# xguo7/SND-VAE

Measured on AMD Instinct MI355X. Metric: training graphs/sec + ELBO-step ms, N=4096 d=64, at 1/2/4/8 MI355X, higher is better.
Workload: dtype bf16; 1 GPU; C2: node-latent SND-VAE train step, N=4096, d=64, 8 graphs/GPU, HIP-graph replay; n_nodes=4096, latent=64, graphs_per_gpu=8, global_batch=8, parallelism=dp1, hip_graph=True

## Files before the change

snd_vae_amd/csrc/snd_fast.hip:

```cpp
#include "snd_fast.hpp"
#include "snd_gather.hpp"
#include "snd_pack.hpp"

#include <algorithm>

namespace snd {

namespace {

constexpr int NT = 256;

typedef short v4s __attribute__((ext_vector_type(4)));
typedef short v8s __attribute__((ext_vector_type(8)));
typedef __attribute__((address_space(3))) v4s lds_v4s;

__device__ __forceinline__ int swz(int row, int kp) {
  return kp >= 128 ? (row & 15) : (kp == 64 ? ((row >> 1) & 7) : 0);
}

__device__ __forceinline__ uint4 pack8(float4 lo, float4 hi) {
  bf16x8 v;
  v[0] = (__bf16)lo.x; v[1] = (__bf16)lo.y; v[2] = (__bf16)lo.z; v[3] = (__bf16)lo.w;
  v[4] = (__bf16)hi.x; v[5] = (__bf16)hi.y; v[6] = (__bf16)hi.z; v[7] = (__bf16)hi.w;
  return __builtin_bit_cast(uint4, v);
}

struct PackPack { PackDesc d[kMaxPack]; };

__global__ void __launch_bounds__(NT) pack_kernel(PackPack pk) {
  const PackDesc& d = pk.d[blockIdx.y];
  const int nch = pack_chunks(d);
  for (int i = blockIdx.x * NT + threadIdx.x; i < nch; i += gridDim.x * NT) pack_chunk(d, i);
}

typedef __attribute__((address_space(1))) const void* gptr_t;
typedef __attribute__((address_space(3))) void* lptr_t;

__device__ __forceinline__ void glds16(const void* g, void* lds_base) {
  __builtin_amdgcn_global_load_lds((gptr_t)g, (lptr_t)lds_base, 16, 0, 0);
}

__device__ __forceinline__ void glds16_async(const void* g, void* lds_base) {
  const unsigned dst = __builtin_amdgcn_readfirstlane((unsigned)(uintptr_t)(lptr_t)lds_base);
  unsigned keep;
  asm volatile("s_mov_b32 %0, m0\n\ts_mov_b32 m0, %2\n\ts_nop 0\n\t"
               "global_load_lds_dwordx4 %1, off\n\ts_mov_b32 m0, %0"
               : "=&s"(keep) : "v"(g), "s"(dst) : "memory");
}

__device__ __forceinline__ int rc_xchunks(int T, int lkc) {
  return (((kRcRows + T - 1) << lkc) + 63) & ~63;
}

constexpr int RCT = 1024;

template <int EPI> struct RcNcp { static constexpr int v = 0; };
template <> struct RcNcp<RC_LIN> { static constexpr int v = 1; };
template <> struct RcNcp<RC_DECBWD> { static constexpr int v = 3; };
template <> struct RcNcp<RC_ENC1> { static constexpr int v = 4; };
template <> struct RcNcp<RC_ENC0> { static constexpr int v = 2; };

template <int EPI, int NBH>
__global__ void __launch_bounds__(RCT) rowconv_kernel(RcArgs a) {
  extern __shared__ __attribute__((aligned(16))) __bf16 lds[];
  __shared__ __attribute__((aligned(16))) float cps[8][RcNcp<EPI>::v > 0 ? RcNcp<EPI>::v : 1][128];
  __shared__ float colp[8][128];
  constexpr int NCP = RcNcp<EPI>::v;
  const int T = a.T, H = (T - 1) >> 1, kp = a.kp, np = a.np;
  const int lkc = kp == 256 ? 5 : (kp == 128 ? 4 : (kp == 64 ? 3 : 2));
  const int XR = kRcRows + T - 1;
  const int xch = rc_xchunks(T, lkc);
  __bf16* xs = lds;
  __bf16* ws = lds + (xch << 3);
  const int tid = threadIdx.x, lane = tid & 63, w = tid >> 6;
  const int li = lane & 15, lg = lane >> 4;
  const int rb = w & 7, nb0 = NBH * (w >> 3);
  int tb = blockIdx.x;
  if (EPI == RC_ENC0 && a.g_rowptr && a.npg % kRcRows == 0 && (a.R / a.npg) % 8 == 0) {
    const int tpg = a.npg / kRcRows, x = tb & 7, sq = tb >> 3, g8 = sq / tpg;
    tb = (x + 8 * g8) * tpg + (sq - g8 * tpg);
  }
  const int r0 = tb * kRcRows;
  const int rend = min(r0 + kRcRows, a.R);
  const int nbase = blockIdx.y * a.npb;
  const int nloc = min(a.npb, np - nbase);
  const int nbc = nloc >> 4;
  const bool use_cp = NCP > 0 && a.colpart != nullptr && !(kdbg(a.dbg) & 64);

  if (!(kdbg(a.dbg) & 1)) {
    const int segc = (nloc * kp) >> 9, npc = T * segc;
    const char* g = reinterpret_cast<const char*>(a.wpk) + lane * 16;
    for (int j = w; j < npc; j += RCT / 64) {
      const int t = j / segc, jj = j - t * segc;
      glds16(g + ((long long)(t * np + nbase) * kp * 2) + (jj << 10), reinterpret_cast<char*>(ws) + (j << 10));
    }
  }
  if (tid < nloc) {
    const int nl = tid, n = nbase + tid;
    const bool cv = n < a.N && a.cols.valid(n) && !(kdbg(a.dbg) & 16);
    const bool pa = n < a.cols.a;
    const int ia = pa ? n : a.cols.logical(n), ib = n - a.cols.offb;
    auto par = [&](const float* A, const float* Bv) {
      return !cv || !A ? 0.f : (pa || !Bv ? A[ia] : Bv[ib]);
    };
    colp[0][nl] = par(a.bias, a.bias_b);
    colp[1][nl] = par(a.gamma, a.gamma_b) * kBnC;
    colp[2][nl] = par(a.beta, a.beta_b);
    if constexpr (EPI == RC_ENC1) {
      colp[3][nl] = (cv && n < a.h) ? a.g2[n] * kBnC : 0.f;
      colp[4][nl] = (cv && n < a.h) ? a.b2[n] : 0.f;
    }
    if constexpr (EPI == RC_ENC0) {
#pragma unroll
      for (int k = 0; k < 4; ++k) colp[3 + k][nl] = (cv && k < a.f) ? a.w0[k * a.N + n] : 0.f;
    }
    if constexpr (EPI == RC_LIN || EPI == RC_FWD) {
#pragma unroll
      for (int k = 0; k < 4; ++k) colp[3 + k][nl] = (cv && k < a.ktail) ? a.wtail[k * a.ldwt + n] : 0.f;
    }
  }

  unsigned cvm[NBH];
#pragma unroll
  for (int i = 0; i < NBH; ++i) {
    cvm[i] = 0u;
#pragma unroll
    for (int e = 0; e < 4; ++e) {
      const int n = nbase + 16 * (nb0 + i) + 4 * lg + e;
      if (nb0 + i < nbc && n < a.N && a.cols.valid(n)) cvm[i] |= 1u << e;
    }
  }
  const int wsw = swz(li, kp);

  int s0 = r0;
  bool first = true;
  while (s0 < rend) {
    int glo, ghi, s1;
    if (T == 1) {
      glo = r0; ghi = rend; s1 = rend;
    } else {
      const int gs = (s0 / a.npg) * a.npg;
      glo = gs; ghi = min(a.R, gs + a.npg); s1 = min(rend, ghi);
    }
    if (!first) __syncthreads();
    bool gathered = false;
    if constexpr (EPI == RC_ENC0 && NBH <= 2) {
      if (a.g_rowptr) {
        gathered = true;
        const int rs = tid >> 3, sub = tid & 7;
        const int gr = r0 + rs;
        float acc8[8] = {0.f, 0.f, 0.f, 0.f, 0.f, 0.f, 0.f, 0.f};
        if (gr < rend) {
          const __amdgpu_buffer_rsrc_t rsx = rows_rsrc(a.x, (long long)a.R * a.ldx * 2);
          gather_rows16<1>(a.g_colidx, a.g_rowptr[gr], a.g_rowptr[gr + 1], rsx, 2u * a.ldx, sub,
                           [&](int, const u32x4 (&v)[1], bool) { acc8v(acc8, v[0]); });
        }
        const uint4 o = to_bf16x8(acc8);
        *reinterpret_cast<uint4*>(xs + rs * kp + ((sub ^ swz(rs, kp)) << 3)) = o;
        if (gr < rend && 8 * sub < a.K)
          *reinterpret_cast<uint4*>(reinterpret_cast<__bf16*>(a.gout) + (long long)gr * a.ldgo + 8 * sub) = o;
      }
    }
    if (!gathered && !(kdbg(a.dbg) & 2)) {
      const int kc = 1 << lkc;
      for (int j = w; j < (xch >> 6); j += RCT / 64) {
        const int q = (j << 6) + lane;
        const int row = q >> lkc, pc = q & (kc - 1);
        const int c = pc ^ swz(row, kp);
        const int gr = r0 - H + row;
        const bool v = row < XR && gr >= glo && gr < ghi && 8 * c < a.K;
        const void* g = v ? (const void*)(reinterpret_cast<const __bf16*>(a.x) + (long long)gr * a.ldx + 8 * c)
                          : (const void*)a.zero;
        glds16(g, reinterpret_cast<char*>(xs) + (j << 10));
      }
    }
    const int r = r0 + 16 * rb + li;
    const bool rv = r >= s0 && r < s1;
    f32x4 ypf[NBH];
#pragma unroll
    for (int i = 0; i < NBH; ++i) ypf[i] = f32x4{0.f, 0.f, 0.f, 0.f};
    if constexpr (EPI == RC_DECBWD || EPI == RC_ENC1) {
      if (rv && !(kdbg(a.dbg) & 32)) {
#pragma unroll
        for (int i = 0; i < NBH; ++i) {
          const int n0 = nbase + 16 * (nb0 + i) + 4 * lg;
          if constexpr (EPI == RC_DECBWD) {
            const float* yp = a.y + (long long)r * a.ldy + n0;
            if (cvm[i] == 15u) ypf[i] = *reinterpret_cast<const f32x4*>(yp);
            else
#pragma unroll
              for (int e = 0; e < 4; ++e) if (cvm[i] >> e & 1u) ypf[i][e] = yp[e];
          } else {
            if (NBH <= 3 && cvm[i] == 15u && n0 + 3 < a.h && (a.ldp & 3) == 0 &&
                (reinterpret_cast<uintptr_t>(a.p) & 15) == 0) {
              ypf[i] = *reinterpret_cast<const f32x4*>(a.p + (long long)r * a.ldp + n0);
            } else {
#pragma unroll
              for (int e = 0; e < 4; ++e) {
                const int n = n0 + e;
                if (cvm[i] >> e & 1u)
                  ypf[i][e] = n < a.h ? a.p[(long long)r * a.ldp + n] : a.xf[(long long)r * a.ldxf + (n - a.h)];
              }
            }
          }
        }
      }
    }
    float ax[4] = {0.f, 0.f, 0.f, 0.f};
    if constexpr (EPI == RC_ENC0) {
      if (rv)
#pragma unroll
        for (int k = 0; k < 4; ++k) if (k < a.f) ax[k] = a.p[(long long)r * a.ldp + k];
    }
    if constexpr (EPI == RC_LIN || EPI == RC_FWD) {
      if (rv && a.ktail > 0) {
        const __bf16* xt = reinterpret_cast<const __bf16*>(a.x) + (long long)r * a.ldx + a.K;
#pragma unroll
        for (int k = 0; k < 4; ++k) if (k < a.ktail) ax[k] = (float)xt[k];
      }
    }
    __builtin_amdgcn_s_waitcnt(0x0F70);
    __syncthreads();

    f32x4 acc[NBH];
#pragma unroll
    for (int i = 0; i < NBH; ++i) acc[i] = f32x4{0.f, 0.f, 0.f, 0.f};
    const int kcs = (kdbg(a.dbg) & 4) ? 0 : kp >> 5;
    for (int t = 0; t < T; ++t) {
      const int xrow = 16 * rb + li + t;
      const __bf16* xrp = xs + xrow * kp;
      const int xsw = swz(xrow, kp);
      const __bf16* wrp = ws + (t * nloc + li) * kp;
      for (int ks = 0; ks < kcs; ++ks) {
        const int ch = 4 * ks + lg;
        const bf16x8 bx = *reinterpret_cast<const bf16x8*>(xrp + ((ch ^ xsw) << 3));
#pragma unroll
        for (int i = 0; i < NBH; ++i) {
          if (nb0 + i < nbc) {
            const bf16x8 aw = *reinterpret_cast<const bf16x8*>(
                wrp + 16 * (nb0 + i) * kp + ((ch ^ wsw) << 3));
            acc[i] = __builtin_amdgcn_mfma_f32_16x16x32_bf16(aw, bx, acc[i], 0, 0, 0);
          }
        }
      }
    }

#pragma unroll
    for (int i = 0; i < NBH; ++i) {
      const int nb = nb0 + i;
      if (nb >= nbc || (kdbg(a.dbg) & 128)) continue;
      const int nl0 = 16 * nb + 4 * lg, n0 = nbase + nl0;
      const unsigned cm = rv ? cvm[i] : 0u;
      float o[4], qs[NCP > 0 ? NCP : 1][4];
#pragma unroll
      for (int q = 0; q < (NCP > 0 ? NCP : 1); ++q)
#pragma unroll
        for (int e = 0; e < 4; ++e) qs[q][e] = 0.f;
      const float4 bia = *reinterpret_cast<const float4*>(&colp[0][nl0]);
      const float4 gam = *reinterpret_cast<const float4*>(&colp[1][nl0]);
      const float4 bet = *reinterpret_cast<const float4*>(&colp[2][nl0]);
      const float bi[4] = {bia.x, bia.y, bia.z, bia.w};
      if constexpr (EPI == RC_LIN || EPI == RC_FWD) {
        if (a.ktail > 0)
#pragma unroll
          for (int e = 0; e < 4; ++e)
#pragma unroll
            for (int k = 0; k < 4; ++k) acc[i][e] += ax[k] * colp[3 + k][nl0 + e];
      }
      const float ga[4] = {gam.x, gam.y, gam.z, gam.w};
      const float be[4] = {bet.x, bet.y, bet.z, bet.w};
      unsigned sm = cm;
      if constexpr (EPI == RC_LIN) {
#pragma unroll
        for (int e = 0; e < 4; ++e) { o[e] = acc[i][e] + bi[e]; qs[0][e] = (cm >> e & 1u) ? o[e] : 0.f; }
      } else if constexpr (EPI == RC_FWD) {
        float yv[4];
#pragma unroll
        for (int e = 0; e < 4; ++e) { yv[e] = acc[i][e] + bi[e]; o[e] = lrelu(yv[e] * ga[e] + be[e]); }
        float* yp = a.y + (long long)r * a.ldy + n0;
        if (kdbg(a.dbg) & 8) {
        } else if (cm == 15u) *reinterpret_cast<float4*>(yp) = make_float4(yv[0], yv[1], yv[2], yv[3]);
        else
#pragma unroll
          for (int e = 0; e < 4; ++e) if (cm >> e & 1u) yp[e] = yv[e];
      } else if constexpr (EPI == RC_DECBWD) {
#pragma unroll
        for (int e = 0; e < 4; ++e) {
          const float yv = ypf[i][e];
          const float dt = (cm >> e & 1u) ? acc[i][e] * lrelu_grad(yv * ga[e] + be[e]) : 0.f;
          o[e] = dt * ga[e];
          qs[0][e] = dt * yv;
          qs[1][e] = dt;
          qs[2][e] = o[e];
        }
      } else if constexpr (EPI == RC_ENC1) {
#pragma unroll
        for (int e = 0; e < 4; ++e) {
          const int n = n0 + e, nl = nl0 + e;
          const bool ok = cm >> e & 1u;
          const float dg = ok ? acc[i][e] : 0.f;
          const bool bpart = n < a.h;
          const float pv = ypf[i][e];
          const float a1 = lrelu(pv);
          const float x2 = bpart ? a1 * colp[3][nl] + colp[4][nl] : pv;
          qs[0][e] = dg * x2;
          qs[1][e] = dg;
          const float dh2 = dg * ga[e];
          o[e] = 0.f;
          qs[2][e] = 0.f;
          qs[3][e] = 0.f;
          if (bpart) {
            qs[2][e] = dh2 * a1;
            qs[3][e] = dh2;
            o[e] = dh2 * colp[3][nl] * lrelu_grad(pv);
          } else {
            sm &= ~(1u << e);
          }
        }
      } else {
#pragma unroll
        for (int e = 0; e < 4; ++e) {
          float pv = 0.f;
#pragma unroll
          for (int k = 0; k < 4; ++k) pv += ax[k] * colp[3 + k][nl0 + e];
          const float db = (cm >> e & 1u) ? acc[i][e] : 0.f;
          qs[0][e] = db * lrelu(pv);
          qs[1][e] = db;
          o[e] = db * ga[e] * lrelu_grad(pv);
        }
      }
      if (kdbg(a.dbg) & 8) sm = 0u;
      if (a.out_bf16) {
        __bf16* op = reinterpret_cast<__bf16*>(a.out) + (long long)r * a.ldo + n0;
        if (sm == 15u) {
          bf16x4 v4;
#pragma unroll
          for (int e = 0; e < 4; ++e) v4[e] = (__bf16)o[e];
          *reinterpret_cast<bf16x4*>(op) = v4;
        } else {
#pragma unroll
          for (int e = 0; e < 4; ++e) if (sm >> e & 1u) op[e] = (__bf16)o[e];
        }
      } else {
        float* op = reinterpret_cast<float*>(a.out) + (long long)r * a.ldo + n0;
        if (sm == 15u) *reinterpret_cast<float4*>(op) = make_float4(o[0], o[1], o[2], o[3]);
        else
#pragma unroll
          for (int e = 0; e < 4; ++e) if (sm >> e & 1u) op[e] = o[e];
      }
      if constexpr (NCP > 0) {
        if (use_cp) {
#pragma unroll
          for (int q = 0; q < NCP; ++q) {
            float v[4];
#pragma unroll
            for (int e = 0; e < 4; ++e) v[e] = row16_sum(qs[q][e]);
            if (li == 0) {
              float4* cp = reinterpret_cast<float4*>(&cps[rb][q][nl0]);
              if (first) *cp = make_float4(v[0], v[1], v[2], v[3]);
              else { float4 o4 = *cp; o4.x += v[0]; o4.y += v[1]; o4.z += v[2]; o4.w += v[3]; *cp = o4; }
            }
          }
        }
      }
    }
    s0 = s1;
    first = false;
  }
  if constexpr (NCP > 0) {
    if (use_cp) {
      __syncthreads();
      for (int i = tid; i < NCP * nloc; i += RCT) {
        const int q = i / nloc, nl = i - q * nloc, n = nbase + nl;
        if (n >= a.N) continue;
        float t = 0.f;
#pragma unroll
        for (int b = 0; b < 8; ++b) t += cps[b][q][nl];
        a.colpart[((long long)tb * NCP + q) * a.N + n] = t;
      }
    }
  }
}

__device__ __forceinline__ bf16x8 tr_pair(const __bf16* p0, const __bf16* p1) {
  const v4s lo = __builtin_amdgcn_ds_read_tr16_b64_v4i16((lds_v4s*)(p0));
  const v4s hi = __builtin_amdgcn_ds_read_tr16_b64_v4i16((lds_v4s*)(p1));
  const v8s c = __builtin_shufflevector(lo, hi, 0, 1, 2, 3, 4, 5, 6, 7);
  return __builtin_bit_cast(bf16x8, c);
}

__device__ __forceinline__ int trsw(int row, int kp) {
  return kp == 128 ? (((row & 3) << 1) | (row & 8))
                   : (kp == 64 ? ((row & 2) | ((row & 8) >> 1)) : (((row >> 3) & 1) << 1));
}
__device__ __forceinline__ int log2kc(int kp) { return kp == 128 ? 4 : (kp == 64 ? 3 : 2); }

__device__ __forceinline__ void stage_tr_image(const __bf16* src, int ld, int K, int base, int nrows,
                                               int vlo, int vhi, int kp, __bf16* dst,
                                               const void* zero) {
  const int lane = threadIdx.x & 63, w = threadIdx.x >> 6;
  const int lk = log2kc(kp), kc = 1 << lk;
  const int npc = ((nrows << lk) + 63) >> 6;
  for (int j = w; j < npc; j += 4) {
    const int q = (j << 6) + lane;
    const int row = q >> lk, pc = q & (kc - 1);
    const int c = pc ^ trsw(row, kp);
    const int gr = base + row;
    const bool v = row < nrows && gr >= vlo && gr < vhi && 8 * c < K;
    const void* g = v ? (const void*)(src + (long long)gr * ld + 8 * c) : zero;
    glds16(g, reinterpret_cast<char*>(dst) + (j << 10));
  }
}

__device__ __forceinline__ int tr_off(int row, int col, int kp) {
  const int c = col >> 3;
  return row * kp + (((c ^ trsw(row, kp)) << 3) | (col & 4));
}

constexpr int WGT = 1024;

__device__ __forceinline__ int cdiv_d(int a, int b) { return (a + b - 1) / b; }

struct WgUnit { int sub, s0, s1, glo, ghi; };

__device__ __forceinline__ WgUnit wg_unit(const WgArgs& a, int sub, int s0, int c1) {
  const int send = min(c1, sub + kRcRows);
  WgUnit u;
  u.sub = sub; u.s0 = s0;
  if (a.T == 1) { u.glo = sub; u.ghi = send; u.s1 = send; }
  else {
    const int gs = (s0 / a.npg) * a.npg;
    u.glo = gs; u.ghi = min(a.R, gs + a.npg); u.s1 = min(send, u.ghi);
  }
  return u;
}

constexpr int kWgStampWords = 12;
__device__ __forceinline__ void wg_stamp(unsigned* ts, int i, bool on) {
  if (on && threadIdx.x == 0 && i < kWgStampWords) ts[i] = (unsigned)__builtin_amdgcn_s_memrealtime();
}

template <int NBO, int NPW = 1>
__device__ __forceinline__ void wgrad_body(const WgArgs& a, const int bx, const int by, __bf16* lds,
                                           unsigned* tsp = nullptr) {
  const bool stamp = tsp != nullptr;
  const int T = a.T, H = (T - 1) >> 1;
  const int XR = kRcRows + T - 1;
  const int kpx = a.K <= 32 ? 32 : (a.K <= 64 ? 64 : 128);
  const int kpy = a.N <= 32 ? 32 : (a.N <= 64 ? 64 : 128);
  const int xch = ((XR << log2kc(kpx)) + 63) & ~63;
  const int bufe = (xch << 3) + kRcRows * kpy;
  const int tid = threadIdx.x, lane = tid & 63, w = __builtin_amdgcn_readfirstlane(tid >> 6);
  const int li = lane & 15, lg = lane >> 4, tq = li >> 2, tp = li & 3;
  const __bf16* xg = reinterpret_cast<const __bf16*>(a.x);
  const __bf16* dg = reinterpret_cast<const __bf16*>(a.dy);
  const int c0 = bx * a.rows_per_wg, c1 = min(a.R, c0 + a.rows_per_wg);
  auto stage = [&](const WgUnit& u, int b) __attribute__((always_inline)) {
    if (kdbg(a.dbg) & 2) return;
    __bf16* xs = lds + b * bufe;
    __bf16* ds = xs + (xch << 3);
    const int lkx = log2kc(kpx), lky = log2kc(kpy);
    const int npx = xch >> 6, npy = (kRcRows << lky) >> 6;
    for (int j = w; j < npx + npy; j += WGT / 64) {
      const bool isx = j < npx;
      const int jj = isx ? j : j - npx;
      const int lk = isx ? lkx : lky, kp = isx ? kpx : kpy;
      const int q = (jj << 6) + lane;
      const int row = q >> lk, pc = q & ((1 << lk) - 1);
      const int c = pc ^ trsw(row, kp);
      const void* g = a.zero;
      if (isx) {
        const int gr = u.sub - H + row;
        if (row < XR && gr >= u.glo && gr < u.ghi && 8 * c < a.K) g = xg + (long long)gr * a.ldx + 8 * c;
      } else {
        const int gr = u.sub + row;
        if (gr >= u.s0 && gr < u.s1 && 8 * c < a.N) g = dg + (long long)gr * a.lddy + 8 * c;
      }
      glds16_async(g, reinterpret_cast<char*>(isx ? xs : ds) + (jj << 10));
    }
  };

  const WgUnit u0 = wg_unit(a, c0, c0, c1);
  if (c0 < c1) stage(u0, 0);
  const int cbn = (a.K + 15) >> 4;
  const int P = T * cbn;
  bool pvs[NPW];
  int ts[NPW], cbs[NPW];
#pragma unroll
  for (int i = 0; i < NPW; ++i) {
    const int wl = w + 16 * i, p = by * a.pairs_per_wg + wl;
    pvs[i] = wl < a.pairs_per_wg && p < P;
    ts[i] = pvs[i] ? p / cbn : 0;
    cbs[i] = pvs[i] ? p - ts[i] * cbn : 0;
  }
  const bool pv = pvs[0];

  f32x4 acc[NPW][NBO];
#pragma unroll
  for (int i = 0; i < NPW; ++i)
#pragma unroll
    for (int j = 0; j < NBO; ++j) acc[i][j] = f32x4{0.f, 0.f, 0.f, 0.f};

  const int rk0 = 8 * lg + tq;
  int xoff[NPW], xoff2[NPW];
#pragma unroll
  for (int i = 0; i < NPW; ++i) {
    xoff[i] = tr_off(rk0 + ts[i], 16 * cbs[i] + 4 * tp, kpx);
    xoff2[i] = tr_off(rk0 + ts[i] + 4, 16 * cbs[i] + 4 * tp, kpx);
  }
  if (kdbg(a.dbg) & 32) return;
  const int doff = rk0 * kpy;
  const int swd = trsw(rk0, kpy), tpl = (4 * tp) & 4, tph = tp >> 1;
  wg_stamp(tsp, 2, stamp);
  if (c0 < c1) {
    WgUnit u = u0;
    for (int k = 0;; ++k) {
      __builtin_amdgcn_s_waitcnt(0x0F70);
      __syncthreads();
      wg_stamp(tsp, 3 + k, stamp && k < 6);
      int nsub = u.sub, ns0 = u.s1;
      if (ns0 >= min(c1, u.sub + kRcRows)) { nsub = u.sub + kRcRows; ns0 = nsub; }
      const bool more = nsub < c1;
      WgUnit un{};
      if (more) { un = wg_unit(a, nsub, ns0, c1); stage(un, (k + 1) & 1); }
      const __bf16* xs = lds + (k & 1) * bufe;
      const __bf16* ds = xs + (xch << 3);
      if (!(kdbg(a.dbg) & 4) && pv) {
#pragma unroll
        for (int ks = 0; ks < kRcRows / 32; ++ks) {
          const __bf16* xb = xs + 32 * ks * kpx;
          const __bf16* db = ds + doff + 32 * ks * kpy;
          bf16x8 bxv[NPW];
#pragma unroll
          for (int i = 0; i < NPW; ++i) bxv[i] = tr_pair(xb + xoff[i], xb + xoff2[i]);
#pragma unroll
          for (int ob = 0; ob < NBO; ++ob) {
            const int dob = (((2 * ob + tph) ^ swd) << 3) | tpl;
            const bf16x8 af = tr_pair(db + dob, db + dob + 4 * kpy);
#pragma unroll
            for (int i = 0; i < NPW; ++i)
              if (i == 0 || pvs[i]) acc[i][ob] = __builtin_amdgcn_mfma_f32_16x16x32_bf16(af, bxv[i], acc[i][ob], 0, 0, 0);
          }
        }
      }
      if (!more) break;
      u = un;
    }
  }
  if (kdbg(a.dbg) & 8) return;
  const int sK = a.sK, sn4 = a.sn4;
#pragma unroll
  for (int i = 0; i < NPW; ++i) {
    const int k = 16 * cbs[i] + li;
    if (!pvs[i] || k >= a.K) continue;
    float* row = a.slab + (long long)bx * T * sK * sn4 + ((long long)ts[i] * sK + a.wk0 + k) * sn4 + a.wn0;
#pragma unroll
    for (int ob = 0; ob < NBO; ++ob) {
      const int n0 = 16 * ob + 4 * lg;
      if (n0 < a.N)
        *reinterpret_cast<float4*>(row + n0) =
            make_float4(acc[i][ob][0], acc[i][ob][1], acc[i][ob][2], acc[i][ob][3]);
    }
  }
}

template <int NBO>
__global__ void __launch_bounds__(WGT) wgrad_kernel(WgArgs a) {
  extern __shared__ __attribute__((aligned(16))) __bf16 lds[];
  wgrad_body<NBO>(a, blockIdx.x, blockIdx.y, lds);
}

struct WgMultiPack {
  WgArgs a[kMaxWgMulti];
  int start[kMaxWgMulti + 1];
  int nseg;
  int stamp_base;
};
static_assert(sizeof(WgMultiPack) <= 4096, "wgrad_multi: kernel arguments over 4 KB");

__global__ void __launch_bounds__(WGT) __attribute__((amdgpu_waves_per_eu(8, 8)))
wgrad_multi_kernel(WgMultiPack m) {
  extern __shared__ __attribute__((aligned(16))) __bf16 lds[];
  __shared__ unsigned tsl[kWgStampWords];
  const bool stamp = (kdbg(m.a[0].dbg) & (1 << 21)) && m.a[0].stamps;
  wg_stamp(tsl, 0, stamp);
  if (kdbg(m.a[0].dbg) & 1) return;
  const int bid = blockIdx.y * gridDim.x + blockIdx.x;
  int s = 0;
  if (gridDim.y > 1) {
    s = blockIdx.y;
  } else {
#pragma unroll
    for (int i = 1; i < kMaxWgMulti; ++i) s += (int)blockIdx.x >= m.start[i] ? 1 : 0;
  }
  s = __builtin_amdgcn_readfirstlane(s);
  const WgArgs a = m.a[s];
  const int local = gridDim.y > 1 ? (int)blockIdx.x : (int)blockIdx.x - m.start[s];
  const int gx = cdiv_d(a.R, a.rows_per_wg);
  const int bx = local % gx, by = local / gx;
  const bool two = a.pairs_per_wg > WGT / 64;
  if (kdbg(a.dbg) & 16) return;
  unsigned* ts = stamp ? tsl : nullptr;
  wg_stamp(ts, 1, stamp);
  switch ((a.N + 15) >> 4) {
    case 1: if (two) wgrad_body<1, 2>(a, bx, by, lds, ts); else wgrad_body<1>(a, bx, by, lds, ts); break;
    case 2: if (two) wgrad_body<2, 2>(a, bx, by, lds, ts); else wgrad_body<2>(a, bx, by, lds, ts); break;
    case 3: if (two) wgrad_body<3, 2>(a, bx, by, lds, ts); else wgrad_body<3>(a, bx, by, lds, ts); break;
    default: if (two) wgrad_body<4, 2>(a, bx, by, lds, ts); else wgrad_body<4>(a, bx, by, lds, ts); break;
  }
  if (stamp) {
    __syncthreads();
    if (threadIdx.x == 0) {
      unsigned* o = m.a[0].stamps + ((long long)m.stamp_base + bid) * kWgStampWords;
      for (int i = 0; i < 9; ++i) o[i] = tsl[i];
      o[9] = (unsigned)__builtin_amdgcn_s_memrealtime();
      o[10] = __builtin_amdgcn_s_getreg((31 << 11) | 4);
      o[11] = __builtin_amdgcn_s_getreg((31 << 11) | 20);
    }
  }
}

struct HeadFastPack { HeadFastArgs h[2]; };

template <int CIN, int COUT>
__device__ __forceinline__ void head_rows(const HeadFastArgs& h, int R) {
  constexpr int NQ = CIN * COUT + COUT + 3 * CIN;
  __shared__ float red[16][NQ];
  __shared__ double sred[4];
  const int tid = threadIdx.x, lane = tid & 63, w = tid >> 6;
  const int r = blockIdx.x * kHeadFastRows + tid;
  const bool rv = r < R;
  float wv[CIN][COUT], bv[COUT], gk[CIN], bk[CIN];
#pragma unroll
  for (int k = 0; k < CIN; ++k) {
#pragma unroll
    for (int o = 0; o < COUT; ++o) wv[k][o] = h.w[k * COUT + o];
    gk[k] = h.gamma[k] * kBnC;
    bk[k] = h.beta[k];
  }
#pragma unroll
  for (int o = 0; o < COUT; ++o) bv[o] = h.b[o];
  float u[CIN], yv[CIN];
#pragma unroll
  for (int k = 0; k < CIN; ++k) { u[k] = 0.f; yv[k] = 0.f; }
  if (rv) {
    if (h.u_bf16) {
      const __bf16* up = reinterpret_cast<const __bf16*>(h.u) + (long long)r * h.ldu;
#pragma unroll
      for (int c = 0; c < (CIN + 7) / 8; ++c) {
        const bf16x8 v = *reinterpret_cast<const bf16x8*>(up + 8 * c);
#pragma unroll
        for (int j = 0; j < 8; ++j) if (8 * c + j < CIN) u[8 * c + j] = (float)v[j];
      }
    } else {
      const float* up = reinterpret_cast<const float*>(h.u) + (long long)r * h.ldu;
#pragma unroll
      for (int c = 0; c < (CIN + 3) / 4; ++c) {
        const float4 v = *reinterpret_cast<const float4*>(up + 4 * c);
        const float vv[4] = {v.x, v.y, v.z, v.w};
#pragma unroll
        for (int j = 0; j < 4; ++j) if (4 * c + j < CIN) u[4 * c + j] = vv[j];
      }
    }
    const float* yp = h.y + (long long)r * h.ldy;
#pragma unroll
    for (int c = 0; c < (CIN + 3) / 4; ++c) {
      const float4 v = *reinterpret_cast<const float4*>(yp + 4 * c);
      const float vv[4] = {v.x, v.y, v.z, v.w};
#pragma unroll
      for (int j = 0; j < 4; ++j) if (4 * c + j < CIN) yv[4 * c + j] = vv[j];
    }
  }
  float tg[COUT];
#pragma unroll
  for (int o = 0; o < COUT; ++o) tg[o] = rv ? h.target[(long long)r * h.ldt + o] : 0.f;
  float dp[COUT];
  double sse = 0.0;
#pragma unroll
  for (int o = 0; o < COUT; ++o) {
    float zo = bv[o];
#pragma unroll
    for (int k = 0; k < CIN; ++k) zo += u[k] * wv[k][o];
    const float yh = 1.f / (1.f + __expf(-zo));
    const float diff = yh - tg[o];
    if (rv) {
      if (h.yhat) h.yhat[(long long)r * COUT + o] = yh;
      sse += (double)diff * diff;
    }
    dp[o] = rv ? 2.f * diff / h.count * yh * (1.f - yh) : 0.f;
  }
  float dt[CIN], dyv[CIN];
#pragma unroll
  for (int k = 0; k < CIN; ++k) {
    float du = 0.f;
#pragma unroll
    for (int o = 0; o < COUT; ++o) du += dp[o] * wv[k][o];
    dt[k] = du * lrelu_grad(yv[k] * gk[k] + bk[k]);
    dyv[k] = dt[k] * gk[k];
  }
  if (rv) {
    __bf16* dq = h.dy + (long long)r * h.lddy;
#pragma unroll
    for (int c = 0; c < CIN / 4; ++c) {
      bf16x4 v;
#pragma unroll
      for (int j = 0; j < 4; ++j) v[j] = (__bf16)dyv[4 * c + j];
      *reinterpret_cast<bf16x4*>(dq + 4 * c) = v;
    }
#pragma unroll
    for (int k = (CIN / 4) * 4; k < CIN; ++k) dq[k] = (__bf16)dyv[k];
  }
  const int grp = 4 * w + (lane >> 4);
  auto put = [&](int q, float v) {
    v = row16_sum(v);
    if ((lane & 15) == 0) red[grp][q] = v;
  };
#pragma unroll
  for (int k = 0; k < CIN; ++k)
#pragma unroll
    for (int o = 0; o < COUT; ++o) put(k * COUT + o, u[k] * dp[o]);
#pragma unroll
  for (int o = 0; o < COUT; ++o) put(CIN * COUT + o, dp[o]);
  constexpr int QB = CIN * COUT + COUT;
#pragma unroll
  for (int k = 0; k < CIN; ++k) {
    put(QB + k, dt[k] * yv[k]);
    put(QB + CIN + k, dt[k]);
    put(QB + 2 * CIN + k, dyv[k]);
  }
  const double wsum = wave_sum_d(sse);
  if (lane == 0) sred[w] = wsum;
  __syncthreads();
  for (int q = tid; q < NQ; q += NT) {
    float t = 0.f;
#pragma unroll
    for (int g = 0; g < 16; ++g) t += red[g][q];
    h.part[(long long)blockIdx.x * NQ + q] = t;
  }
  if (tid == 0) h.sse[blockIdx.x] = sred[0] + sred[1] + sred[2] + sred[3];
}

__global__ void __launch_bounds__(NT) heads_fast_kernel(HeadFastPack pk, int R) {
  const HeadFastArgs& h = pk.h[blockIdx.y];
  if (h.cin == 10 && h.cout == 2) head_rows<10, 2>(h, R);
  else if (h.cin == 20 && h.cout == 1) head_rows<20, 1>(h, R);
}

template <int EPI>
int rc_launch_epi(const RcArgs& a, hipStream_t s) {
  const size_t lds = rc_lds_bytes(a.T, a.kp, a.npb);
  const dim3 grid(rc_blocks(a.R), cdiv(a.np, a.npb)), block(RCT);
  switch ((a.npb / 16 + 1) / 2) {
    case 1: hipLaunchKernelGGL((rowconv_kernel<EPI, 1>), grid, block, lds, s, a); break;
    case 2: hipLaunchKernelGGL((rowconv_kernel<EPI, 2>), grid, block, lds, s, a); break;
    case 3: hipLaunchKernelGGL((rowconv_kernel<EPI, 3>), grid, block, lds, s, a); break;
    default: hipLaunchKernelGGL((rowconv_kernel<EPI, 4>), grid, block, lds, s, a); break;
  }
  SND_LAUNCH_CHECK("rowconv_kernel");
  return 0;
}

int kp_img(int k) { return k <= 32 ? 32 : (k <= 64 ? 64 : 128); }
size_t wg_lds_bytes(int T, int K, int N) {
  const int kpx = kp_img(K), kpy = kp_img(N);
  const size_t xch = round_up((long long)(kRcRows + T - 1) * (kpx / 8), 64);
  return 2 * (xch * 8 + (size_t)kRcRows * kpy) * 2;
}

template <int NBO>
int wg_launch(const WgArgs& a, dim3 grid, hipStream_t s) {
  hipLaunchKernelGGL((wgrad_kernel<NBO>), grid, dim3(WGT), wg_lds_bytes(a.T, a.K, a.N), s, a);
  SND_LAUNCH_CHECK("wgrad_kernel");
  return 0;
}

constexpr size_t kMaxDynLds = kRcLdsLimit;
constexpr size_t kWgMultiLds = 128 * 1024;

}

size_t pack_bytes(int T, int kp, int np) { return (size_t)T * kp * np * 2; }

int launch_pack(const PackDesc* d, int n, hipStream_t s) {
  if (n < 1 || n > kMaxPack) { set_error("pack: 1..%d descriptors", kMaxPack); return SND_ERR_ARG; }
  PackPack pk{};
  int maxch = 0;
  for (int i = 0; i < n; ++i) {
    const PackDesc& x = d[i];
    if (!(x.kp == 32 || x.kp == 64 || x.kp == 128 || x.kp == 256) || x.np % 16 || x.np <= 0 || x.T < 1 ||
        x.nsrc < 1 || x.nsrc > 2) {
      set_error("pack: bad descriptor %d (kp %d np %d T %d)", i, x.kp, x.np, x.T);
      return SND_ERR_ARG;
    }
    pk.d[i] = x;
    maxch = std::max(maxch, x.T * x.np * x.kp / 8);
  }
  dim3 grid(cdiv(maxch, NT), n);
  hipLaunchKernelGGL(pack_kernel, grid, dim3(NT), 0, s, pk);
  SND_LAUNCH_CHECK("pack_kernel");
  return 0;
}

int rc_blocks(int R) { return cdiv(R, kRcRows); }

int heads_fast_blocks(int R) { return cdiv(R, kHeadFastRows); }
bool heads_fast_supported(int cin, int cout) { return (cin == 10 && cout == 2) || (cin == 20 && cout == 1); }
int heads_fast_parts(int cin, int cout) { return cin * cout + cout + 3 * cin; }

int launch_heads_fast(const HeadFastArgs* h, int n, int R, hipStream_t s) {
  if (n < 1 || n > 2) { set_error("heads_fast: 1 or 2 heads"); return SND_ERR_ARG; }
  HeadFastPack pk{};
  for (int i = 0; i < n; ++i) {
    const HeadFastArgs& x = h[i];
    SND_CHECK_ARG(heads_fast_supported(x.cin, x.cout), "heads_fast: (cin, cout) = (%d, %d) not built",
                  x.cin, x.cout);
    SND_CHECK_ARG(x.ldu >= (int)round_up(x.cin, x.u_bf16 ? 8 : 4) && x.ldy >= (int)round_up(x.cin, 4) &&
                      x.ldu % (x.u_bf16 ? 8 : 4) == 0 && x.ldy % 4 == 0,
                  "heads_fast: padded leading dims required");
    SND_CHECK_ARG(x.u && x.y && x.gamma && x.beta && x.w && x.b && x.target && x.dy && x.part && x.sse,
                  "heads_fast: null operand");
    pk.h[i] = x;
  }
  if (R <= 0) return 0;
  hipLaunchKernelGGL(heads_fast_kernel, dim3(heads_fast_blocks(R), n), dim3(NT), 0, s, pk, R);
  SND_LAUNCH_CHECK("heads_fast_kernel");
  return 0;
}

size_t rc_lds_bytes(int T, int kp, int np) {
  const size_t xch = round_up((long long)(kRcRows + T - 1) * (kp / 8), 64);
  return (xch * 8 + (size_t)T * np * kp) * 2;
}

#ifndef SND_RC_FILL
#define SND_RC_FILL 256
#endif
int rc_cols_per_block(int T, int kp, int np) {
  for (int s = cdiv(np, 128); s <= 8; ++s) {
    const int npb = (int)round_up(cdiv(np, s), 16);
    if (npb <= 128 && rc_lds_bytes(T, kp, npb) <= kMaxDynLds) return npb;
  }
  return 0;
}

int launch_rowconv(const RcArgs& a0, int epi, hipStream_t s) {
  if (a0.R <= 0) return 0;
  RcArgs a = a0;
  SND_CHECK_ARG(a.T == 1 || a.T == 5, "rowconv: T must be 1 or 5");
  SND_CHECK_ARG(a.kp == 32 || a.kp == 64 || a.kp == 128 || a.kp == 256, "rowconv: kp %d", a.kp);
  SND_CHECK_ARG(a.ktail == 0 || ((epi == RC_LIN || epi == RC_FWD) && a.ktail <= 4 && a.wtail && a.ldwt >= a.N &&
                                 a.cols.b == 0),
                "rowconv: K tail needs RC_LIN / RC_FWD, <= 4 columns, a plain layout");
  SND_CHECK_ARG(a.np % 16 == 0 && a.np >= 16 && a.np <= 256, "rowconv: np %d", a.np);
  SND_CHECK_ARG(a.K <= a.kp && a.N <= a.np && a.N > 0, "rowconv: K %d / N %d exceed image", a.K, a.N);
  SND_CHECK_ARG(a.ldx % 8 == 0 && a.ldo % 4 == 0, "rowconv: ldx %% 8 / ldo %% 4");
  a.npb = rc_cols_per_block(a.T, a.kp, a.np);
  SND_CHECK_ARG(a.npb > 0, "rowconv: LDS image too large (T %d kp %d np %d)", a.T, a.kp, a.np);
  for (;;) {
    const int nb = (int)round_up(cdiv(a.npb, 2), 16);
    if ((a.dbg & (1 << 19)) || a.g_rowptr || rc_blocks(a.R) * cdiv(a.np, a.npb) >= SND_RC_FILL || nb < 32 ||
        nb >= a.npb) break;
    a.npb = nb;
  }
  SND_CHECK_ARG(a.x && a.wpk && a.out && a.zero && a.x_bf16, "rowconv: null operand / fp32 x");
  SND_CHECK_ARG(!a.colpart || (a.ncp >= 1 && a.ncp <= 4), "rowconv: ncp");
  SND_CHECK_ARG(a.npg > 0, "rowconv: npg");
  SND_CHECK_ARG(!a.g_rowptr || (epi == RC_ENC0 && a.T == 1 && a.kp == 64 && a.K <= 64 && a.np <= 64 && a.g_colidx &&
                                a.gout && a.ldgo % 8 == 0 && a.ldx % 8 == 0 && a.npb == a.np),
                "rowconv: the gathered x rows need RC_ENC0, T 1, kp 64, one column window");
  switch (epi) {
    case RC_LIN: return rc_launch_epi<RC_LIN>(a, s);
    case RC_FWD:
      SND_CHECK_ARG(a.y && a.bias && a.gamma && a.beta && a.ldy % 4 == 0, "rowconv fwd: BN operands");
      return rc_launch_epi<RC_FWD>(a, s);
    case RC_DECBWD:
      SND_CHECK_ARG(a.y && a.gamma && a.beta && a.ldy % 4 == 0, "rowconv decbwd: BN operands");
      return rc_launch_epi<RC_DECBWD>(a, s);
    case RC_ENC1:
      SND_CHECK_ARG(a.p && a.xf && a.gamma && a.g2 && a.b2 && a.h % 4 == 0, "rowconv enc1 operands");
      return rc_launch_epi<RC_ENC1>(a, s);
    case RC_ENC0:
      SND_CHECK_ARG(a.p && a.w0 && a.gamma && a.f <= 4, "rowconv enc0 operands");
      return rc_launch_epi<RC_ENC0>(a, s);
    default: set_error("rowconv: bad epilogue %d", epi); return SND_ERR_ARG;
  }
}

static WgArgs wg_norm(const WgArgs& a) {
  WgArgs x = a;
  if (x.sK == 0) { x.sK = x.K; x.sn4 = wgrad_n4(x.N); x.wk0 = 0; x.wn0 = 0; }
  return x;
}

#ifndef SND_WG_SPLIT_LDS
#define SND_WG_SPLIT_LDS (80 * 1024)
#endif
constexpr size_t kWgSplitLds = SND_WG_SPLIT_LDS;
static int wg_split(const WgArgs& a, WgArgs* out, int cap) {
  const bool sk = a.K > 64 && wg_lds_bytes(a.T, a.K, std::min(a.N, 64)) > kWgSplitLds, sn = a.N > 64;
  int n = 0;
  for (int k0 = 0; k0 < a.K; k0 += sk ? 64 : a.K)
    for (int n0 = 0; n0 < a.N; n0 += sn ? 64 : a.N) {
      if (n >= cap) return -1;
      WgArgs w = a;
      w.K = sk ? std::min(64, a.K - k0) : a.K;
      w.N = sn ? std::min(64, a.N - n0) : a.N;
      w.x = static_cast<const __bf16*>(a.x) + k0;
      w.dy = static_cast<const __bf16*>(a.dy) + n0;
      w.wk0 = a.wk0 + k0; w.wn0 = a.wn0 + n0;
      w.pairs_per_wg = std::min(a.pairs_per_wg, a.T * cdiv(w.K, 16));
      out[n++] = w;
    }
  return n;
}

static int wg_multi_flush(WgMultiPack& pk, int total, size_t lds, hipStream_t s) {
  if (pk.nseg == 0) return 0;
  for (int i = pk.nseg; i <= kMaxWgMulti; ++i) pk.start[i] = total;
  bool uniform = pk.nseg > 1;
  for (int i = 1; i < pk.nseg; ++i) uniform = uniform && pk.start[i + 1] - pk.start[i] == pk.start[1];
  const dim3 grid = uniform ? dim3(pk.start[1], pk.nseg) : dim3(total);
  hipLaunchKernelGGL(wgrad_multi_kernel, grid, dim3(WGT), lds, s, pk);
  SND_LAUNCH_CHECK("wgrad_multi_kernel");
  return 0;
}

int launch_wgrad_multi(const WgArgs* a, int n, hipStream_t s) {
  if (n <= 0) return 0;
  WgMultiPack pk{};
  size_t lds = 0;
  int total = 0, base = 0;
  pk.nseg = 0;
  const bool stamps = a[0].stamps != nullptr;
  for (int i = 0; i < n; ++i) {
    const WgArgs x0 = wg_norm(a[i]);
    if (x0.R <= 0) continue;
    SND_CHECK_ARG(x0.T == 1 || x0.T == 5, "wgrad_multi: T must be 1 or 5");
    SND_CHECK_ARG(x0.K > 0 && x0.K <= 128 && x0.N > 0 && x0.N <= 128, "wgrad_multi: K %d N %d", x0.K, x0.N);
    SND_CHECK_ARG(x0.ldx % 8 == 0 && x0.lddy % 8 == 0 && x0.x_bf16 && x0.dy_bf16,
                  "wgrad_multi: bf16 operands with leading dims %% 8");
    SND_CHECK_ARG(x0.rows_per_wg % kRcRows == 0 && x0.pairs_per_wg >= 1 && x0.pairs_per_wg <= 2 * WGT / 64,
                  "wgrad_multi: geometry");
    SND_CHECK_ARG(x0.x && x0.dy && x0.slab && x0.zero && x0.npg > 0, "wgrad_multi: null operand");
    SND_CHECK_ARG(x0.sn4 % 4 == 0 && x0.wn0 % 4 == 0 && x0.wk0 + x0.K <= x0.sK &&
                  x0.wn0 + wgrad_n4(x0.N) <= x0.sn4, "wgrad_multi: slab window");
    WgArgs win[4];
    const int nw = wg_split(x0, win, 4);
    SND_CHECK_ARG(nw > 0, "wgrad_multi: window split");
    for (int j = 0; j < nw; ++j) {
      if (pk.nseg == kMaxWgMulti) {
        SND_TRY(wg_multi_flush(pk, total, lds, s));
        base += total;
        pk = WgMultiPack{};
        pk.stamp_base = base;
        lds = 0;
        total = 0;
      }
      const WgArgs& x = win[j];
      const int P = x.T * cdiv(x.K, 16);
      pk.a[pk.nseg] = x;
      pk.start[pk.nseg] = total;
      total += cdiv(x.R, x.rows_per_wg) * cdiv(P, x.pairs_per_wg);
      lds = std::max(lds, wg_lds_bytes(x.T, x.K, x.N));
      ++pk.nseg;
      SND_CHECK_ARG(!stamps || ((long long)base + total) * kWgStampWords <= a[0].stamp_words,
                    "wgrad_multi: %d workgroups' stamps exceed the %lld-word buffer", base + total,
                    a[0].stamp_words);
    }
  }
  return wg_multi_flush(pk, total, lds, s);
}

WgGeom wgrad_geom(int R, int T, int K, int N, int chunks) {
  WgGeom g{};
  const int P = T * cdiv(K, 16);
  g.pairs_per_wg = std::min(P, WGT / 64);
  g.gy = cdiv(P, g.pairs_per_wg);
  if (chunks > 0) {
    g.pairs_per_wg = std::min(P, 2 * WGT / 64);
    g.gy = cdiv(P, g.pairs_per_wg);
    g.rows_per_wg = (int)round_up(cdiv(R, chunks), kRcRows);
    g.gx = cdiv(R, g.rows_per_wg);
    return g;
  }
  int gx = std::max(1, 256 / g.gy);
  if ((long long)T * K * N >= 65536) gx = std::min(gx, 64);
  g.rows_per_wg = (int)round_up(cdiv(R, gx), kRcRows);
  g.gx = cdiv(R, g.rows_per_wg);
  return g;
}

int launch_wgrad(const WgArgs& a0, hipStream_t s) {
  const WgArgs a = wg_norm(a0);
  if (a.R <= 0) return 0;
  SND_CHECK_ARG(a.T == 1 || a.T == 5, "wgrad: T must be 1 or 5");
  SND_CHECK_ARG(a.K > 0 && a.K <= 128 && a.N > 0 && a.N <= 128, "wgrad: K %d N %d", a.K, a.N);
  SND_CHECK_ARG(a.ldx % 8 == 0 && a.lddy % 8 == 0 && a.x_bf16 && a.dy_bf16,
                "wgrad: bf16 operands with leading dims %% 8");
  SND_CHECK_ARG(a.rows_per_wg % kRcRows == 0 && a.pairs_per_wg >= 1 && a.pairs_per_wg <= WGT / 64,
                "wgrad: geometry");
  SND_CHECK_ARG(a.x && a.dy && a.slab && a.zero && a.npg > 0, "wgrad: null operand");
  const int P = a.T * cdiv(a.K, 16);
  dim3 grid(cdiv(a.R, a.rows_per_wg), cdiv(P, a.pairs_per_wg));
  switch (cdiv(a.N, 16)) {
    case 1: return wg_launch<1>(a, grid, s);
    case 2: return wg_launch<2>(a, grid, s);
    case 3: return wg_launch<3>(a, grid, s);
    case 4: return wg_launch<4>(a, grid, s);
    case 5: return wg_launch<5>(a, grid, s);
    case 6: return wg_launch<6>(a, grid, s);
    case 7: return wg_launch<7>(a, grid, s);
    default: return wg_launch<8>(a, grid, s);
  }
}

static thread_local int g_dbg = 0;
int debug_flags() { return g_dbg; }

static int fast_init_attributes_once() {
#define SND_ATTR(K)                                                                       \
  if (hipFuncSetAttribute(reinterpret_cast<const void*>(K),                               \
                          hipFuncAttributeMaxDynamicSharedMemorySize, (int)kMaxDynLds) != \
      hipSuccess) {                                                                       \
    set_error("hipFuncSetAttribute(%s) failed", #K);                                      \
    return SND_ERR_HIP;                                                                   \
  }
#define SND_ATTR4(E) SND_ATTR((rowconv_kernel<E, 1>)) SND_ATTR((rowconv_kernel<E, 2>)) \
                     SND_ATTR((rowconv_kernel<E, 3>)) SND_ATTR((rowconv_kernel<E, 4>))
  SND_ATTR4(RC_LIN) SND_ATTR4(RC_FWD) SND_ATTR4(RC_DECBWD) SND_ATTR4(RC_ENC1) SND_ATTR4(RC_ENC0)
#undef SND_ATTR4
  SND_ATTR((wgrad_kernel<1>)) SND_ATTR((wgrad_kernel<2>)) SND_ATTR((wgrad_kernel<3>))
  SND_ATTR((wgrad_kernel<4>)) SND_ATTR((wgrad_kernel<5>)) SND_ATTR((wgrad_kernel<6>))
  SND_ATTR((wgrad_kernel<7>)) SND_ATTR((wgrad_kernel<8>))
#undef SND_ATTR
  if (hipFuncSetAttribute(reinterpret_cast<const void*>(wgrad_multi_kernel),
                          hipFuncAttributeMaxDynamicSharedMemorySize, (int)kWgMultiLds) != hipSuccess) {
    set_error("hipFuncSetAttribute(wgrad_multi_kernel) failed");
    return SND_ERR_HIP;
  }
  return 0;
}

int fast_init_attributes() {
  static const int rc = fast_init_attributes_once();
  return rc;
}

}

extern "C" int snd_debug_set(int flags) {
  snd::g_dbg = flags;
  return 0;
}
```

snd_vae_amd/csrc/snd_gather.hpp:

```cpp
#pragma once
#include "snd_common.hpp"

namespace snd {

constexpr int kLpr = 8;

typedef unsigned u32x4 __attribute__((ext_vector_type(4)));
typedef __bf16 gbf16x2 __attribute__((ext_vector_type(2)));

__device__ __forceinline__ float dot8_bf16(const u32x4& a, const u32x4& b, float acc) {
  const unsigned wa[4] = {a.x, a.y, a.z, a.w}, wb[4] = {b.x, b.y, b.z, b.w};
#pragma unroll
  for (int p = 0; p < 4; ++p)
    acc = __builtin_amdgcn_fdot2_f32_bf16(__builtin_bit_cast(gbf16x2, wa[p]), __builtin_bit_cast(gbf16x2, wb[p]),
                                          acc, false);
  return acc;
}

template <int U>
__device__ __forceinline__ int bcast8(int v) {
  return __builtin_amdgcn_ds_swizzle(v, 0x18 | (U << 5));
}

__device__ __forceinline__ __amdgpu_buffer_rsrc_t rows_rsrc(const void* base, long long bytes) {
  return __builtin_amdgcn_make_buffer_rsrc(const_cast<void*>(base), 0, (int)bytes, 0x00020000);
}

template <int NQ, typename Fn>
__device__ __forceinline__ void gather_rows16(const int* colidx, int s, int e, __amdgpu_buffer_rsrc_t rs,
                                              unsigned row_bytes, int sub, Fn&& fn) {
  for (int k0 = s; k0 < e; k0 += 16) {
    const int id0 = k0 + sub < e ? colidx[k0 + sub] : -1;
    const int id1 = k0 + 8 + sub < e ? colidx[k0 + 8 + sub] : -1;
    int c[16];
    c[0] = bcast8<0>(id0); c[1] = bcast8<1>(id0); c[2] = bcast8<2>(id0); c[3] = bcast8<3>(id0);
    c[4] = bcast8<4>(id0); c[5] = bcast8<5>(id0); c[6] = bcast8<6>(id0); c[7] = bcast8<7>(id0);
    c[8] = bcast8<0>(id1); c[9] = bcast8<1>(id1); c[10] = bcast8<2>(id1); c[11] = bcast8<3>(id1);
    c[12] = bcast8<4>(id1); c[13] = bcast8<5>(id1); c[14] = bcast8<6>(id1); c[15] = bcast8<7>(id1);
    u32x4 v[16][NQ];
#pragma unroll
    for (int u = 0; u < 16; ++u) {
      const unsigned off = (unsigned)c[u] * row_bytes + 16u * sub;
#pragma unroll
      for (int q = 0; q < NQ; ++q) v[u][q] = __builtin_amdgcn_raw_buffer_load_b128(rs, off + 128u * q, 0, 0);
    }
    __builtin_amdgcn_sched_barrier(0);
    const int nv = e - k0;
#pragma unroll
    for (int u = 0; u < 16; ++u) fn(u, v[u], u < nv);
  }
}

__device__ __forceinline__ void acc8v(float (&a)[8], const u32x4& v) {
  unsigned lo1u, hi1u;
  asm volatile("s_mov_b32 %0, 0x3f80" : "=s"(lo1u));
  asm volatile("s_mov_b32 %0, 0x3f800000" : "=s"(hi1u));
  const gbf16x2 lo1 = __builtin_bit_cast(gbf16x2, lo1u);
  const gbf16x2 hi1 = __builtin_bit_cast(gbf16x2, hi1u);
  const unsigned w[4] = {v.x, v.y, v.z, v.w};
#pragma unroll
  for (int p = 0; p < 4; ++p) {
    const gbf16x2 x = __builtin_bit_cast(gbf16x2, w[p]);
    a[2 * p] = __builtin_amdgcn_fdot2_f32_bf16(x, lo1, a[2 * p], false);
    a[2 * p + 1] = __builtin_amdgcn_fdot2_f32_bf16(x, hi1, a[2 * p + 1], false);
  }
}

__device__ __forceinline__ void widen8(float (&a)[8], const u32x4& v) {
#pragma unroll
  for (int p = 0; p < 4; ++p) {
    const unsigned w = v[p];
    a[2 * p] = __uint_as_float(w << 16);
    a[2 * p + 1] = __uint_as_float(w & 0xFFFF0000u);
  }
}

__device__ __forceinline__ uint4 to_bf16x8(const float (&v)[8]) {
  bf16x8 o;
#pragma unroll
  for (int j = 0; j < 8; ++j) o[j] = (__bf16)v[j];
  return __builtin_bit_cast(uint4, o);
}

}
```

snd_vae_amd/csrc/snd_head.hip:

```cpp
#include "snd_head.hpp"
#include "snd_gather.hpp"
#include "snd_pack.hpp"

#include <algorithm>

namespace snd {
namespace {

constexpr int kHeadRows = 64;
constexpr int HWMAX = 16;
constexpr float kSqrtLog2e = 1.2011224087864498f;
__device__ __forceinline__ int cdiv_dev(int a, int b) { return (a + b - 1) / b; }

typedef __attribute__((address_space(1))) const void* gptr_t;
typedef __attribute__((address_space(3))) void* lptr_t;

__device__ __forceinline__ void hglds16(const void* g, void* lds) {
  __builtin_amdgcn_global_load_lds((gptr_t)g, (lptr_t)lds, 16, 0, 0);
}
__host__ __device__ __forceinline__ int hswz(int row, int kp) {
  return kp == 128 ? (row & 15) : (kp == 64 ? ((row >> 1) & 7) : 0);
}

struct FwdLay {
  int w2, w1, g, h, zt, total, sx_end;
  __host__ __device__ FwdLay(int HR, int kp1, int np1, int kp2, int np2, int L) {
    w2 = 0;
    w1 = np2 * kp2 * 2;
    g = w1 + np1 * kp1 * 2;
    h = g + HR * kp1 * 2;
    zt = h + HR * kp2 * 2;
    total = zt + HR * (L + 1) * 4;
    sx_end = 2 * HR * (L + 4) * 4;
  }
};
constexpr int kHeadStaticLds = 2 * 128 * 4 + 2 * HWMAX * 8;
constexpr int kHeadDynLds = 160 * 1024 - kHeadStaticLds - 512;

__device__ __forceinline__ void stage_img(const __bf16* src, int bytes, char* dst, int nw) {
  const int lane = threadIdx.x & 63, w = threadIdx.x >> 6;
  const char* g = reinterpret_cast<const char*>(src) + lane * 16;
  for (int j = w; j < (bytes >> 10); j += nw) hglds16(g + (j << 10), dst + (j << 10));
}

template <int NBH>
__device__ __forceinline__ void img_gemm(const __bf16* xs, const __bf16* ws, int kp, int np, int rb,
                                         int nb0, int li, int lg, f32x4 (&acc)[NBH]) {
  const int nbc = np >> 4;
#pragma unroll
  for (int i = 0; i < NBH; ++i) acc[i] = f32x4{0.f, 0.f, 0.f, 0.f};
  const int xrow = 16 * rb + li;
  const __bf16* xrp = xs + xrow * kp;
  const int xsw = hswz(xrow, kp), wsw = hswz(li, kp);
  const __bf16* wrp = ws + li * kp;
  const int kcs = kp >> 5;
  for (int ks = 0; ks < kcs; ++ks) {
    const int ch = 4 * ks + lg;
    const bf16x8 bx = *reinterpret_cast<const bf16x8*>(xrp + ((ch ^ xsw) << 3));
#pragma unroll
    for (int i = 0; i < NBH; ++i) {
      if (nb0 + i < nbc) {
        const bf16x8 aw = *reinterpret_cast<const bf16x8*>(wrp + 16 * (nb0 + i) * kp + ((ch ^ wsw) << 3));
        acc[i] = __builtin_amdgcn_mfma_f32_16x16x32_bf16(aw, bx, acc[i], 0, 0, 0);
      }
    }
  }
}

__device__ __forceinline__ bf16x4* img_at4(__bf16* img, int row, int n0, int kp) {
  return reinterpret_cast<bf16x4*>(img + row * kp + (((n0 >> 3) ^ hswz(row, kp)) << 3) + (n0 & 4));
}

template <int HR, int NB1, int NB2>
__global__ void __launch_bounds__(HR * 8) head_fwd_kernel(HeadFwdArgs a) {
  constexpr int HT = HR * 8, HW = HT / 64, NRB = HR / 16;
  extern __shared__ __attribute__((aligned(16))) char smem[];
  __shared__ float cb1[128], cb2[128];
  __shared__ double klw[2 * HWMAX];
  const FwdLay lay(HR, a.kp1, a.np1, a.kp2, a.np2, a.L);
  __bf16* w2s = reinterpret_cast<__bf16*>(smem + lay.w2);
  __bf16* w1s = reinterpret_cast<__bf16*>(smem + lay.w1);
  __bf16* gs = reinterpret_cast<__bf16*>(smem + lay.g);
  __bf16* hs = reinterpret_cast<__bf16*>(smem + lay.h);
  float* mx = reinterpret_cast<float*>(smem);
  float* sx = reinterpret_cast<float*>(smem + HR * (a.L + 4) * 4);
  float* zt = reinterpret_cast<float*>(smem + lay.zt);
  const int L = a.L, sxs = L + 4, zts = L + 1;
  const int tid = threadIdx.x, lane = tid & 63, w = tid >> 6;
  const int tpg = a.npad / HR;
  int tb = blockIdx.x;
  if (a.ngraphs % 8 == 0 && a.ngraphs > 0) {
    const int x = tb & 7, sq = tb >> 3;
    const int g8 = sq / tpg;
    tb = (x + 8 * g8) * tpg + (sq - g8 * tpg);
  }
  const int gi = tb / tpg, lt = tb - gi * tpg;
  const int lr0 = lt * HR;
  const long long gr0 = (long long)gi * a.npg;

  stage_img(a.wh_img, a.np1 * a.kp1 * 2, reinterpret_cast<char*>(w1s), HW);
  stage_img(a.wms_img, a.np2 * a.kp2 * 2, reinterpret_cast<char*>(w2s), HW);
  for (int i = tid; i < 128; i += HT) {
    cb1[i] = i < a.gh ? a.bh[i] : 0.f;
    cb2[i] = i < 2 * L ? a.bms[i] : 0.f;
  }
  for (int i = tid; i < HR * a.kp2 / 8; i += HT) reinterpret_cast<uint4*>(hs)[i] = make_uint4(0u, 0u, 0u, 0u);

  const int rs = tid >> 3, sub = tid & 7;
  const int lr = lr0 + rs;
  const bool rv = lr < a.npg;
  const long long r = gr0 + lr;
  float acc[8];
#pragma unroll
  for (int j = 0; j < 8; ++j) acc[j] = 0.f;
  if (rv && !(kdbg(a.dbg) & 1)) {
    const __amdgpu_buffer_rsrc_t rsd = rows_rsrc(a.xw1, (long long)a.R * a.h1 * 2);
    gather_rows16<1>(a.colidx, a.rowptr[r], a.rowptr[r + 1], rsd, 2u * a.h1, sub,
                     [&](int, const u32x4 (&v)[1], bool) { acc8v(acc, v[0]); });
  }
  const int nch = a.h1 >> 3, kc1 = a.kp1 >> 3;
  uint4 gdat = make_uint4(0u, 0u, 0u, 0u), gxv = make_uint4(0u, 0u, 0u, 0u);
  if (sub < nch) {
    float gv[8];
#pragma unroll
    for (int j = 0; j < 8; ++j) {
      const int c = 8 * sub + j;
      const float b1 = lrelu(acc[j]) * (a.g1[c] * kBnC) + a.b1[c];
      gv[j] = b1 * (a.ge[c] * kBnC) + a.be[c];
    }
    gdat = to_bf16x8(gv);
  }
  const int xo = (sub == nch) ? 0 : (sub + 8 == nch ? 1 : -1);
  if (xo >= 0 && rv) {
    float gv[8];
#pragma unroll
    for (int j = 0; j < 8; ++j) {
      const int c = a.h1 + j;
      gv[j] = j < a.f ? a.x[r * a.ldx + j] * (a.ge[c] * kBnC) + a.be[c] : 0.f;
    }
    gxv = to_bf16x8(gv);
  }
  {
    const bool d0 = sub < nch, x0 = xo == 0, x1 = xo == 1;
    const uint4 v0 = make_uint4(d0 ? gdat.x : (x0 ? gxv.x : 0u), d0 ? gdat.y : (x0 ? gxv.y : 0u),
                                d0 ? gdat.z : (x0 ? gxv.z : 0u), d0 ? gdat.w : (x0 ? gxv.w : 0u));
    const uint4 v1 = make_uint4(x1 ? gxv.x : 0u, x1 ? gxv.y : 0u, x1 ? gxv.z : 0u, x1 ? gxv.w : 0u);
    if (sub < kc1) *reinterpret_cast<uint4*>(gs + rs * a.kp1 + ((sub ^ hswz(rs, a.kp1)) << 3)) = v0;
    if (sub + 8 < kc1) *reinterpret_cast<uint4*>(gs + rs * a.kp1 + (((sub + 8) ^ hswz(rs, a.kp1)) << 3)) = v1;
  }
  __builtin_amdgcn_s_waitcnt(0x0F70);
  __syncthreads();
  if (rv && !(kdbg(a.dbg) & 8)) {
    if (sub < nch) {
      float* pp = a.p1 + r * a.h1 + 8 * sub;
      *reinterpret_cast<float4*>(pp) = make_float4(acc[0], acc[1], acc[2], acc[3]);
      *reinterpret_cast<float4*>(pp + 4) = make_float4(acc[4], acc[5], acc[6], acc[7]);
      *reinterpret_cast<uint4*>(a.g + r * a.ldg + 8 * sub) = gdat;
    }
    if (xo >= 0) *reinterpret_cast<uint4*>(a.g + r * a.ldg + a.h1) = gxv;
  }

  const int li = lane & 15, lg = lane >> 4, rb = w % NRB, half = w / NRB;
  const int row = 16 * rb + li, lrw = lr0 + row;
  const bool vrow = lrw < a.npg;
  const long long rr = gr0 + lrw;
  {
    f32x4 acc1[NB1];
    if (kdbg(a.dbg) & 16) { for (int i = 0; i < NB1; ++i) acc1[i] = f32x4{0.f, 0.f, 0.f, 0.f}; }
    else img_gemm<NB1>(gs, w1s, a.kp1, a.np1, rb, NB1 * half, li, lg, acc1);
#pragma unroll
    for (int i = 0; i < NB1; ++i) {
      const int n0 = 16 * (NB1 * half + i) + 4 * lg;
      if (n0 >= a.gh) continue;
      bf16x4 v4;
#pragma unroll
      for (int e = 0; e < 4; ++e) v4[e] = (__bf16)(acc1[i][e] + cb1[n0 + e]);
      *img_at4(hs, row, n0, a.kp2) = v4;
      if (vrow && !(kdbg(a.dbg) & 8)) *reinterpret_cast<bf16x4*>(a.hh + rr * a.gh + n0) = v4;
    }
  }
  __syncthreads();

  {
    f32x4 acc2[NB2];
    if (kdbg(a.dbg) & 16) { for (int i = 0; i < NB2; ++i) acc2[i] = f32x4{0.f, 0.f, 0.f, 0.f}; }
    else img_gemm<NB2>(hs, w2s, a.kp2, a.np2, rb, NB2 * half, li, lg, acc2);
    float o[NB2][4];
#pragma unroll
    for (int i = 0; i < NB2; ++i) {
      const int n0 = 16 * (NB2 * half + i) + 4 * lg;
#pragma unroll
      for (int e = 0; e < 4; ++e) o[i][e] = acc2[i][e] + cb2[n0 + e];
      if (vrow && !(kdbg(a.dbg) & 8))
        *reinterpret_cast<float4*>(a.ms + rr * (2 * L) + n0) = make_float4(o[i][0], o[i][1], o[i][2], o[i][3]);
    }
    __syncthreads();
#pragma unroll
    for (int i = 0; i < NB2; ++i) {
      const int n0 = 16 * (NB2 * half + i) + 4 * lg;
      *reinterpret_cast<float4*>((half ? sx : mx) + row * sxs + (n0 - half * L)) =
          make_float4(o[i][0], o[i][1], o[i][2], o[i][3]);
    }
  }
  __syncthreads();

  {
    const unsigned off = a.step ? (unsigned)(*a.step) : 0u;
    if (a.stepn && blockIdx.x == 0 && tid == 0) *a.stepn = (int)off + 1;
    const int nq = L >> 2;
    double kl[HR / 64];
#pragma unroll
    for (int h = 0; h < HR / 64; ++h) kl[h] = 0.0;
    for (int it = (kdbg(a.dbg) & 32) ? HR * nq : tid; it < HR * nq; it += HT) {
      const int zr = it / nq, c = 4 * (it - zr * nq);
      const int zl = lr0 + zr;
      float z4[4] = {0.f, 0.f, 0.f, 0.f};
      if (zl < a.npg) {
        const long long ie = (gr0 + zl) * L + c;
        const float4 m4 = *reinterpret_cast<const float4*>(mx + zr * sxs + c);
        const float4 s4 = *reinterpret_cast<const float4*>(sx + zr * sxs + c);
        const float4 ep = a.eps_in ? *reinterpret_cast<const float4*>(a.eps_in + ie)
                                   : philox_normal4(a.seed, off, (a.eps_base + (unsigned long long)ie) >> 2);
        const float mu[4] = {m4.x, m4.y, m4.z, m4.w}, s[4] = {s4.x, s4.y, s4.z, s4.w};
        const float e[4] = {ep.x, ep.y, ep.z, ep.w};
        double kq = 0.0;
#pragma unroll
        for (int t = 0; t < 4; ++t) {
          const float es = __expf(s[t]);
          z4[t] = mu[t] + e[t] * es;
          kq += (double)kl_elem(s[t], mu[t]);
        }
#pragma unroll
        for (int h = 0; h < HR / 64; ++h) kl[h] += (zr >> 6) == h ? kq : 0.0;
        if (!(kdbg(a.dbg) & 8)) {
          *reinterpret_cast<float4*>(a.z + ie) = make_float4(z4[0], z4[1], z4[2], z4[3]);
          *reinterpret_cast<float4*>(a.eps_out + ie) = ep;
          bf16x4 zb;
#pragma unroll
          for (int t = 0; t < 4; ++t) zb[t] = (__bf16)z4[t];
          *reinterpret_cast<bf16x4*>(a.zb + ie) = zb;
        }
      }
      bf16x4 jb;
#pragma unroll
      for (int t = 0; t < 4; ++t) {
        jb[t] = (__bf16)(z4[t] * kSqrtLog2e);
        zt[zr * zts + c + t] = z4[t];
      }
      *reinterpret_cast<bf16x4*>(a.jrow + ((long long)gi * a.npad + zl) * L + c) = jb;
    }
#pragma unroll
    for (int h = 0; h < HR / 64; ++h) {
      const double v = wave_sum_d(kl[h]);
      if (lane == 0) klw[h * HWMAX + w] = v;
    }
  }
  __syncthreads();
  for (int i = (kdbg(a.dbg) & 64) ? HT * HR : tid; i < (HR / 64) * L; i += HT) {
    const int h = i / L, c = i - h * L;
    float cs = 0.f;
    for (int q0 = 0; q0 < 64; q0 += 16) {
      float t[16];
#pragma unroll
      for (int u = 0; u < 16; ++u) t[u] = zt[(64 * h + q0 + u) * zts + c];
#pragma unroll
      for (int u = 0; u < 16; ++u) cs += (float)(__bf16)(t[u] * kSqrtLog2e);
    }
    a.colpart[((long long)gi * (a.npad / 64) + (HR / 64) * lt + h) * L + c] = cs;
  }
  for (int idx = (kdbg(a.dbg) & 64) ? HT * HR : tid; idx < (HR / 4) * L; idx += HT) {
    const int c = idx / (HR / 4), r4 = 4 * (idx % (HR / 4));
    bf16x4 t;
#pragma unroll
    for (int u = 0; u < 4; ++u) t[u] = (__bf16)zt[(r4 + u) * zts + c];
    *reinterpret_cast<bf16x4*>(a.jt + ((long long)gi * L + c) * a.npad + lr0 + r4) = t;
  }
  if (tid < HR / 64) {
    double v = 0.0;
    for (int k = 0; k < HW; ++k) v += klw[tid * HWMAX + k];
    a.kl_part[(long long)gi * (a.npad / 64) + (HR / 64) * lt + tid] = v;
  }
}

template <int HR, int NB1, int NB2>
int head_fwd_launch(const HeadFwdArgs& a, hipStream_t s) {
  const size_t lds = (size_t)FwdLay(HR, a.kp1, a.np1, a.kp2, a.np2, a.L).total;
  hipLaunchKernelGGL((head_fwd_kernel<HR, NB1, NB2>), dim3(a.ngraphs * (a.npad / HR)), dim3(HR * 8), lds, s, a);
  SND_LAUNCH_CHECK("head_fwd_kernel");
  return 0;
}
template <int HR>
int head_fwd_dispatch(const HeadFwdArgs& a, hipStream_t s) {
  const int nb1 = (a.np1 / 16 + 1) / 2, nb2 = a.np2 / 32;
  if (nb1 == 1) return nb2 == 2 ? head_fwd_launch<HR, 1, 2>(a, s) : head_fwd_launch<HR, 1, 4>(a, s);
  return nb2 == 2 ? head_fwd_launch<HR, 2, 2>(a, s) : head_fwd_launch<HR, 2, 4>(a, s);
}

struct BwdLay {
  int w1, w2, m, h, red, total;
  __host__ __device__ BwdLay(int kp1, int np1, int kp2, int np2, int L, int hr = kHeadBwdRows) {
    w1 = 0;
    w2 = np1 * kp1 * 2;
    m = w2 + np2 * kp2 * 2;
    h = m + hr * kp1 * 2;
    red = h + hr * kp2 * 2;
    total = red + (hr / 8) * 2 * L * 4;
  }
};
constexpr int kBwdStaticLds = ((kHeadBwdRows / 16) * 4 * 128 + (kHeadBwdRows / 16) * 128 + 5 * 128) * 4 +
                              (kHeadBwdRows / 8) * 12;

__device__ __forceinline__ float shfl_rows8(float v) {
  v += __shfl_xor(v, 8, 64);
  v += __shfl_xor(v, 16, 64);
  v += __shfl_xor(v, 32, 64);
  return v;
}

template <int HR, int NQ, int NB1, int NB2>
__global__ void __launch_bounds__(HR * 8) head_bwd_kernel(HeadBwdArgs a) {
  constexpr int HT = HR * 8, HW = HT / 64, NRB = HR / 16;
  extern __shared__ __attribute__((aligned(16))) char smem[];
  __shared__ __attribute__((aligned(16))) float cps[NRB][4][128];
  __shared__ __attribute__((aligned(16))) float cpb[NRB][128];
  __shared__ float colp[5][128];
  __shared__ double sl[HW];
  __shared__ unsigned stp[HW];
  const BwdLay lay(a.kp1, a.np1, a.kp2, a.np2, a.L, HR);
  __bf16* w1s = reinterpret_cast<__bf16*>(smem + lay.w1);
  __bf16* w2s = reinterpret_cast<__bf16*>(smem + lay.w2);
  __bf16* ms_img = reinterpret_cast<__bf16*>(smem + lay.m);
  __bf16* dh_img = reinterpret_cast<__bf16*>(smem + lay.h);
  float* bred = reinterpret_cast<float*>(smem + lay.red);
  const int L = a.L, L2 = 2 * L;
  const int tid = threadIdx.x, lane = tid & 63, w = tid >> 6;
  int t = blockIdx.x;
  if (a.ngraphs % 8 == 0 && a.npg % HR == 0 && a.ngraphs > 0) {
    const int tpg = a.npg / HR, x = t & 7, sq = t >> 3;
    const int gi = sq / tpg;
    t = (x + 8 * gi) * tpg + (sq - gi * tpg);
  }
  const int r0 = t * HR;

  stage_img(a.wmsb_img, a.np1 * a.kp1 * 2, reinterpret_cast<char*>(w1s), HW);
  stage_img(a.whb_img, a.np2 * a.kp2 * 2, reinterpret_cast<char*>(w2s), HW);
  for (int i = tid; i < HR * a.kp2 / 8; i += HT) reinterpret_cast<uint4*>(dh_img)[i] = make_uint4(0u, 0u, 0u, 0u);
  for (int n = tid; n < 128; n += HT) {
    const bool cv = n < a.W;
    colp[1][n] = cv ? a.ge[n] * kBnC : 0.f;
    colp[3][n] = (cv && n < a.h1) ? a.g1[n] * kBnC : 0.f;
    colp[4][n] = (cv && n < a.h1) ? a.b1[n] : 0.f;
  }

  {
    const int rs = tid >> 3, sub = tid & 7;
    const int r = r0 + rs;
    const bool rv = r < a.R;
    const int nch = L >> 3;
    bool qv[NQ];
#pragma unroll
    for (int q = 0; q < NQ; ++q) qv[q] = sub + 8 * q < nch;
    float lossr = 0.f;
    unsigned tp = 0;
    u32x4 zi[NQ];
    float ej[NQ][8];
#pragma unroll
    for (int q = 0; q < NQ; ++q) {
      zi[q] = u32x4{0u, 0u, 0u, 0u};
#pragma unroll
      for (int j = 0; j < 8; ++j) ej[q][j] = 0.f;
    }
    if (rv)
#pragma unroll
      for (int q = 0; q < NQ; ++q)
        if (qv[q]) zi[q] = *reinterpret_cast<const u32x4*>(a.zb + (long long)r * L + 64 * q + 8 * sub);
    const float pw = a.pos_weight;
    if (rv && !(kdbg(a.dbg) & 1)) {
      const __amdgpu_buffer_rsrc_t rsd = rows_rsrc(a.zb, (long long)a.R * L * 2);
      gather_rows16<NQ>(a.colidx, a.rowptr[r], a.rowptr[r + 1], rsd, 2u * L, sub,
                        [&](int, const u32x4 (&v)[NQ], bool valid) {
        float zj[NQ][8], dot = 0.f;
#pragma unroll
        for (int q = 0; q < NQ; ++q)
#pragma unroll
          for (int p = 0; p < 4; ++p) {
            const unsigned wv = v[q][p];
            zj[q][2 * p] = qv[q] ? __uint_as_float(wv << 16) : 0.f;
            zj[q][2 * p + 1] = qv[q] ? __uint_as_float(wv & 0xFFFF0000u) : 0.f;
          }
#pragma unroll
        for (int q = 0; q < NQ; ++q)
          if (qv[q]) dot = dot8_bf16(zi[q], v[q], dot);
        const float Lij = row8_sum(dot);
        if (!valid) return;
        float coef;
        edge_ce_terms(Lij, pw, coef, lossr);
        lossr -= pw * Lij;
        tp += Lij > 0.f ? 1u : 0u;
#pragma unroll
        for (int q = 0; q < NQ; ++q)
#pragma unroll
          for (int j = 0; j < 8; ++j) ej[q][j] += coef * zj[q][j];
      });
    }
    if (sub != 0 || !rv) { lossr = 0.f; tp = 0; }
    float dm[NQ][8], dl[NQ][8];
#pragma unroll
    for (int q = 0; q < NQ; ++q) {
#pragma unroll
      for (int j = 0; j < 8; ++j) { dm[q][j] = 0.f; dl[q][j] = 0.f; }
      const int c0 = 64 * q + 8 * sub;
      if (rv && qv[q]) {
        const float* msr = a.ms + (long long)r * L2;
        const long long ie = (long long)r * L + c0;
#pragma unroll
        for (int h = 0; h < 2; ++h) {
          const float4 mu = *reinterpret_cast<const float4*>(msr + c0 + 4 * h);
          const float4 ls = *reinterpret_cast<const float4*>(msr + L + c0 + 4 * h);
          const float4 ep = *reinterpret_cast<const float4*>(a.eps + ie + 4 * h);
          float4 dj = *reinterpret_cast<const float4*>(a.dJd + ie + 4 * h);
          for (int sx = 0; sx < a.nextra; ++sx) {
            const float4 e = *reinterpret_cast<const float4*>(a.dJd_extra + (long long)sx * a.R * L + ie + 4 * h);
            dj.x += e.x; dj.y += e.y; dj.z += e.z; dj.w += e.w;
          }
          const float4 dd = *reinterpret_cast<const float4*>(a.dz_dec + ie + 4 * h);
          const float m4[4] = {mu.x, mu.y, mu.z, mu.w}, l4[4] = {ls.x, ls.y, ls.z, ls.w};
          const float e4[4] = {ep.x, ep.y, ep.z, ep.w}, j4[4] = {dj.x, dj.y, dj.z, dj.w};
          const float d4[4] = {dd.x, dd.y, dd.z, dd.w};
#pragma unroll
          for (int u = 0; u < 4; ++u)
            reparam_bwd_elem(m4[u], l4[u], e4[u], j4[u], ej[q][4 * h + u], d4[u], a.adj_scale, a.kl_scale,
                             dm[q][4 * h + u], dl[q][4 * h + u]);
        }
      }
      if (qv[q]) {
        bf16x8 om, os;
#pragma unroll
        for (int j = 0; j < 8; ++j) { om[j] = (__bf16)dm[q][j]; os[j] = (__bf16)dl[q][j]; }
        const int cm = c0 >> 3, cs = (L + c0) >> 3;
        *reinterpret_cast<bf16x8*>(ms_img + rs * a.kp1 + ((cm ^ hswz(rs, a.kp1)) << 3)) = om;
        *reinterpret_cast<bf16x8*>(ms_img + rs * a.kp1 + ((cs ^ hswz(rs, a.kp1)) << 3)) = os;
        if (rv && !(kdbg(a.dbg) & 8)) {
          *reinterpret_cast<bf16x8*>(a.dms + (long long)r * L2 + c0) = om;
          *reinterpret_cast<bf16x8*>(a.dms + (long long)r * L2 + L + c0) = os;
        }
#pragma unroll
        for (int j = 0; j < 8; ++j) {
          const float sm = shfl_rows8(dm[q][j]), ss = shfl_rows8(dl[q][j]);
          if (lane < 8) { bred[w * L2 + c0 + j] = sm; bred[w * L2 + L + c0 + j] = ss; }
        }
      }
    }
    const double lw = wave_sum_d((double)lossr);
    const unsigned tw = wave_sum_u(tp);
    if (lane == 0) { sl[w] = lw; stp[w] = tw; }
  }
  __builtin_amdgcn_s_waitcnt(0x0F70);
  __syncthreads();
  if (tid < L2) {
    float v = 0.f;
    for (int k = 0; k < HW; ++k) v += bred[k * L2 + tid];
    a.bms_part[(long long)t * L2 + tid] = v;
  }
  if (tid == 0) {
    double tl = 0.0, tt = 0.0;
    for (int k = 0; k < HW; ++k) { tl += sl[k]; tt += (double)stp[k]; }
    a.edge_part[2 * t] = tl;
    a.edge_part[2 * t + 1] = tt;
  }

  const int li = lane & 15, lg = lane >> 4, rb = w % NRB, half = w / NRB;
  const int row = 16 * rb + li, r = r0 + row;
  const bool vrow = r < a.R;
  {
    f32x4 acc1[NB1];
    img_gemm<NB1>(ms_img, w1s, a.kp1, a.np1, rb, NB1 * half, li, lg, acc1);
#pragma unroll
    for (int i = 0; i < NB1; ++i) {
      const int nb = NB1 * half + i;
      if (nb >= (a.np1 >> 4)) continue;
      const int n0 = 16 * nb + 4 * lg;
      const bool cv = vrow && n0 < a.gh;
      float qs[4];
      bf16x4 v4;
#pragma unroll
      for (int e = 0; e < 4; ++e) {
        const float o = acc1[i][e] + 0.f;
        qs[e] = cv ? o : 0.f;
        v4[e] = (__bf16)o;
      }
      if (n0 < a.gh) *img_at4(dh_img, row, n0, a.kp2) = v4;
      if (cv && !(kdbg(a.dbg) & 8)) *reinterpret_cast<bf16x4*>(a.dh + (long long)r * a.gh + n0) = v4;
#pragma unroll
      for (int e = 0; e < 4; ++e) qs[e] = row16_sum(qs[e]);
      if (li == 0) *reinterpret_cast<float4*>(&cpb[rb][n0]) = make_float4(qs[0], qs[1], qs[2], qs[3]);
    }
  }
  f32x4 ypf[NB2];
  unsigned cvm[NB2];
#pragma unroll
  for (int i = 0; i < NB2; ++i) {
    ypf[i] = f32x4{0.f, 0.f, 0.f, 0.f};
    cvm[i] = 0u;
    const int nb = NB2 * half + i;
#pragma unroll
    for (int e = 0; e < 4; ++e) {
      const int n = 16 * nb + 4 * lg + e;
      if (nb < (a.np2 >> 4) && n < a.W) {
        cvm[i] |= 1u << e;
        if (vrow) ypf[i][e] = n < a.h1 ? a.p1[(long long)r * a.h1 + n] : a.x[(long long)r * a.ldx + (n - a.h1)];
      }
    }
  }
  __syncthreads();
  if (tid < a.gh) {
    float v = 0.f;
#pragma unroll
    for (int b = 0; b < NRB; ++b) v += cpb[b][tid];
    a.bh_part[(long long)t * a.gh + tid] = v;
  }

  {
    f32x4 acc2[NB2];
    img_gemm<NB2>(dh_img, w2s, a.kp2, a.np2, rb, NB2 * half, li, lg, acc2);
#pragma unroll
    for (int i = 0; i < NB2; ++i) {
      const int nb = NB2 * half + i;
      if (nb >= (a.np2 >> 4)) continue;
      const int n0 = 16 * nb + 4 * lg;
      const unsigned cm = vrow ? cvm[i] : 0u;
      unsigned sm = cm;
      float o[4], qs[4][4];
#pragma unroll
      for (int e = 0; e < 4; ++e) {
        const int n = n0 + e;
        const bool ok = cm >> e & 1u;
        const float dg = ok ? acc2[i][e] : 0.f;
        const bool bpart = n < a.h1;
        const float pv = ypf[i][e];
        const float a1 = lrelu(pv);
        const float x2 = bpart ? a1 * colp[3][n] + colp[4][n] : pv;
        qs[0][e] = dg * x2;
        qs[1][e] = dg;
        const float dh2 = dg * colp[1][n];
        o[e] = 0.f;
        qs[2][e] = 0.f;
        qs[3][e] = 0.f;
        if (bpart) {
          qs[2][e] = dh2 * a1;
          qs[3][e] = dh2;
          o[e] = dh2 * colp[3][n] * lrelu_grad(pv);
        } else {
          sm &= ~(1u << e);
        }
      }
      if (!(kdbg(a.dbg) & 8)) {
        __bf16* op = a.dp1 + (long long)r * a.h1 + n0;
        if (sm == 15u) {
          bf16x4 v4;
#pragma unroll
          for (int e = 0; e < 4; ++e) v4[e] = (__bf16)o[e];
          *reinterpret_cast<bf16x4*>(op) = v4;
        } else {
#pragma unroll
          for (int e = 0; e < 4; ++e) if (sm >> e & 1u) op[e] = (__bf16)o[e];
        }
      }
#pragma unroll
      for (int q = 0; q < 4; ++q) {
        float v[4];
#pragma unroll
        for (int e = 0; e < 4; ++e) v[e] = row16_sum(qs[q][e]);
        if (li == 0) *reinterpret_cast<float4*>(&cps[rb][q][n0]) = make_float4(v[0], v[1], v[2], v[3]);
      }
    }
  }
  __syncthreads();
  for (int i = tid; i < 4 * a.W; i += HT) {
    const int q = i / a.W, n = i - q * a.W;
    float v = 0.f;
#pragma unroll
    for (int b = 0; b < NRB; ++b) v += cps[b][q][n];
    a.enc1_part[(long long)t * 4 * a.W + i] = v;
  }
}

template <int NQ, int NB1, int NB2>
int head_bwd_launch(const HeadBwdArgs& a, hipStream_t s) {
  const int hr = head_bwd_rows(a.R);
  const size_t lds = (size_t)BwdLay(a.kp1, a.np1, a.kp2, a.np2, a.L, hr).total;
  if (hr == kHeadBwdTinyRows)
    hipLaunchKernelGGL((head_bwd_kernel<kHeadBwdTinyRows, NQ, NB1, NB2>), dim3(head_tiles(a.R)),
                       dim3(kHeadBwdTinyRows * 8), lds, s, a);
  else if (hr == 64)
    hipLaunchKernelGGL((head_bwd_kernel<64, NQ, NB1, NB2>), dim3(head_tiles(a.R)), dim3(64 * 8), lds, s, a);
  else
    hipLaunchKernelGGL((head_bwd_kernel<kHeadBwdRows, NQ, NB1, NB2>), dim3(head_tiles(a.R)),
                       dim3(kHeadBwdRows * 8), lds, s, a);
  SND_LAUNCH_CHECK("head_bwd_kernel");
  return 0;
}

template <int NB>
__global__ void __launch_bounds__(1024) enc_front_kernel(FrontArgs a) {
  const int tid = threadIdx.x;
  const int ntiles = cdiv_dev(a.R, 128);
  if ((int)blockIdx.x >= ntiles) {
    const int pb = blockIdx.x - ntiles;
    int s = 0;
    while (s + 1 < a.npack && pb >= a.pack_wg[s + 1]) ++s;
    s = __builtin_amdgcn_readfirstlane(s);
    const PackDesc& d = a.pack[s];
    const int i = (pb - a.pack_wg[s]) * 1024 + tid;
    if (i < pack_chunks(d)) pack_chunk(d, i);
    return;
  }
  extern __shared__ __attribute__((aligned(16))) char smem[];
  __shared__ float sp[6][128];
  __bf16* wimg = reinterpret_cast<__bf16*>(smem);
  __bf16* himg = reinterpret_cast<__bf16*>(smem + a.np1 * a.kp1 * 2);
  const int r0 = blockIdx.x * 128;
  const int K1 = a.h0 + a.f;
  for (int i = tid; i < a.h0; i += 1024) {
#pragma unroll
    for (int q = 0; q < 4; ++q) sp[q][i] = q < a.f ? a.w0[q * a.h0 + i] : 0.f;
    sp[4][i] = a.g0[i] * kBnC;
    sp[5][i] = a.b0[i];
  }
  __syncthreads();
  const int kc = a.kp1 >> 3;
  const bool w1one = a.np1 * kc <= 1024;
  float w1v[8];
  if (w1one && tid < a.np1 * kc) {
    const int c = tid % kc, n = tid / kc;
    const int lc = c ^ img_swz(n, a.kp1);
#pragma unroll
    for (int j = 0; j < 8; ++j) {
      const int k = 8 * lc + j;
      w1v[j] = (k < K1 && n < a.n1) ? a.w1[k * a.n1 + n] : 0.f;
    }
  }
  const int rs = tid >> 3, sub = tid & 7;
  const int r = r0 + rs;
  const bool rv = r < a.R;
  float ax[4] = {0.f, 0.f, 0.f, 0.f};
  if (rv) {
    const int s = a.rowptr[r], e = a.rowptr[r + 1];
    int k = s + sub;
    for (; k + 8 < e; k += 16) {
      const int c0 = a.colidx[k], c1 = a.colidx[k + 8];
      float v0[4], v1[4];
#pragma unroll
      for (int j = 0; j < 4; ++j) {
        v0[j] = j < a.f ? a.x[(long long)c0 * a.ldx + j] : 0.f;
        v1[j] = j < a.f ? a.x[(long long)c1 * a.ldx + j] : 0.f;
      }
#pragma unroll
      for (int j = 0; j < 4; ++j) ax[j] += v0[j] + v1[j];
    }
    if (k < e) {
      const int c0 = a.colidx[k];
#pragma unroll
      for (int j = 0; j < 4; ++j) ax[j] += j < a.f ? a.x[(long long)c0 * a.ldx + j] : 0.f;
    }
  }
#pragma unroll
  for (int j = 0; j < 4; ++j) ax[j] = row8_sum(ax[j]);
  const int nch = a.h0 >> 3, kc1 = a.kp1 >> 3;
  uint4 hd = make_uint4(0u, 0u, 0u, 0u), hx = make_uint4(0u, 0u, 0u, 0u);
  if (sub < nch) {
    float o[8];
#pragma unroll
    for (int j = 0; j < 8; ++j) {
      const int col = 8 * sub + j;
      float p = 0.f;
#pragma unroll
      for (int q = 0; q < 4; ++q) p += ax[q] * sp[q][col];
      o[j] = lrelu(p) * sp[4][col] + sp[5][col];
    }
    hd = to_bf16x8(o);
  }
  const int xo = (sub == nch) ? 0 : (sub + 8 == nch ? 1 : -1);
  if (xo >= 0 && rv) {
    float xv[8];
#pragma unroll
    for (int j = 0; j < 8; ++j) xv[j] = j < a.f ? a.x[(long long)r * a.ldx + j] : 0.f;
    hx = to_bf16x8(xv);
  }
  {
    const bool d0 = sub < nch, x0 = xo == 0, x1 = xo == 1;
    const uint4 v0 = make_uint4(d0 ? hd.x : (x0 ? hx.x : 0u), d0 ? hd.y : (x0 ? hx.y : 0u),
                                d0 ? hd.z : (x0 ? hx.z : 0u), d0 ? hd.w : (x0 ? hx.w : 0u));
    const uint4 v1 = make_uint4(x1 ? hx.x : 0u, x1 ? hx.y : 0u, x1 ? hx.z : 0u, x1 ? hx.w : 0u);
    if (sub < kc1) *reinterpret_cast<uint4*>(himg + rs * a.kp1 + ((sub ^ hswz(rs, a.kp1)) << 3)) = v0;
    if (sub + 8 < kc1) *reinterpret_cast<uint4*>(himg + rs * a.kp1 + (((sub + 8) ^ hswz(rs, a.kp1)) << 3)) = v1;
  }
  if (w1one) {
    if (tid < a.np1 * kc) {
      const int c = tid % kc, n = tid / kc;
      bf16x8 v;
#pragma unroll
      for (int j = 0; j < 8; ++j) v[j] = (__bf16)w1v[j];
      *reinterpret_cast<bf16x8*>(wimg + n * a.kp1 + 8 * c) = v;
    }
  } else {
    for (int i = tid; i < a.np1 * kc; i += 1024) {
      const int c = i % kc, n = i / kc;
      const int lc = c ^ img_swz(n, a.kp1);
      bf16x8 v;
#pragma unroll
      for (int j = 0; j < 8; ++j) {
        const int k = 8 * lc + j;
        v[j] = (__bf16)((k < K1 && n < a.n1) ? a.w1[k * a.n1 + n] : 0.f);
      }
      *reinterpret_cast<bf16x8*>(wimg + n * a.kp1 + 8 * c) = v;
    }
  }
  if (rv && !(kdbg(a.dbg) & 8)) {
    if (sub < nch) *reinterpret_cast<uint4*>(a.h1 + (long long)r * a.ldh1 + 8 * sub) = hd;
    if (xo >= 0) *reinterpret_cast<uint4*>(a.h1 + (long long)r * a.ldh1 + a.h0) = hx;
    if (sub == 0) {
      *reinterpret_cast<float4*>(a.ax + (long long)r * 4) = make_float4(ax[0], ax[1], ax[2], ax[3]);
      const float axp[8] = {ax[0], ax[1], ax[2], ax[3], 0.f, 0.f, 0.f, 0.f};
      *reinterpret_cast<uint4*>(a.axb + (long long)r * 8) = to_bf16x8(axp);
    }
  }
  __syncthreads();
  const int lane = tid & 63, w = tid >> 6;
  const int li = lane & 15, lg = lane >> 4, rb = w & 7, half = w >> 3;
  const int row = 16 * rb + li, rr = r0 + row;
  f32x4 acc[NB];
  img_gemm<NB>(himg, wimg, a.kp1, a.np1, rb, NB * half, li, lg, acc);
  if (rr >= a.R || (kdbg(a.dbg) & 8)) return;
#pragma unroll
  for (int i = 0; i < NB; ++i) {
    const int n0 = 16 * (NB * half + i) + 4 * lg;
    if (n0 >= a.n1) continue;
    bf16x4 v4;
#pragma unroll
    for (int e = 0; e < 4; ++e) v4[e] = (__bf16)(acc[i][e] + 0.f);
    *reinterpret_cast<bf16x4*>(a.xw1 + (long long)rr * a.n1 + n0) = v4;
  }
}

}

bool front_supported(int f, int h0, int n1, int kp1, int np1) {
  return f >= 1 && f <= 4 && h0 % 8 == 0 && h0 >= 8 && h0 <= 64 && h0 + 8 <= kp1 && n1 % 16 == 0 &&
         np1 == n1 && np1 <= 128 && (kp1 == 32 || kp1 == 64 || kp1 == 128) &&
         (np1 + 128) * kp1 * 2 + 6 * 128 * 4 <= 160 * 1024;
}

int launch_front(FrontArgs& a, const PackDesc* pack, int npack, hipStream_t s) {
  if (a.R <= 0) return 0;
  SND_CHECK_ARG(front_supported(a.f, a.h0, a.n1, a.kp1, a.np1), "front: unsupported widths (f %d h0 %d n1 %d)",
                a.f, a.h0, a.n1);
  SND_CHECK_ARG(npack >= 0 && npack <= kMaxPack, "front: at most %d packed images", kMaxPack);
  SND_CHECK_ARG(a.rowptr && (a.colidx || a.R == 0) && a.x && a.w0 && a.g0 && a.b0 && a.h1 && a.ax && a.axb &&
                    a.w1 && a.xw1 && a.ldh1 % 8 == 0 && a.ldh1 >= a.h0 + 8,
                "front: operands");
  a.npack = npack;
  int wg = 0;
  for (int i = 0; i < npack; ++i) {
    const PackDesc& x = pack[i];
    SND_CHECK_ARG((x.kp == 32 || x.kp == 64 || x.kp == 128) && x.np % 16 == 0 && x.np > 0 && x.T >= 1 &&
                      x.nsrc >= 1 && x.nsrc <= 2,
                  "front: bad pack descriptor %d", i);
    a.pack[i] = x;
    a.pack_wg[i] = wg;
    wg += cdiv(pack_chunks(x), 1024);
  }
  a.pack_wg[npack] = wg;
  SND_TRY(head_init_attributes());
  const size_t lds = (size_t)(a.np1 + 128) * a.kp1 * 2;
  const dim3 grid(cdiv(a.R, 128) + wg);
  switch ((a.np1 / 16 + 1) / 2) {
    case 1: hipLaunchKernelGGL((enc_front_kernel<1>), grid, dim3(1024), lds, s, a); break;
    case 2: hipLaunchKernelGGL((enc_front_kernel<2>), grid, dim3(1024), lds, s, a); break;
    case 3: hipLaunchKernelGGL((enc_front_kernel<3>), grid, dim3(1024), lds, s, a); break;
    default: hipLaunchKernelGGL((enc_front_kernel<4>), grid, dim3(1024), lds, s, a); break;
  }
  SND_LAUNCH_CHECK("enc_front_kernel");
  return 0;
}

int head_bwd_rows(int R) {
  if (cdiv(R, kHeadBwdRows) >= kHeadBwdSmall) return kHeadBwdRows;
  return cdiv(R, 64) < kHeadBwdTiny ? kHeadBwdTinyRows : 64;
}
int head_tiles(int R) { return cdiv(R, head_bwd_rows(R)); }

bool head_bwd_supported(int L, int gh, int W, int h1, int kp1, int np1, int kp2, int np2) {
  if ((L != 16 && L != 32 && L != 64) || kp1 != 2 * L) return false;
  if (gh % 16 || gh < 16 || np1 != gh || np1 > 64 || gh > kp2 || (kp2 != 32 && kp2 != 64 && kp2 != 128)) return false;
  if (W > 128 || np2 != (int)round_up(W, 16) || h1 % 4 || h1 > W) return false;
  return BwdLay(kp1, np1, kp2, np2, L).total + kBwdStaticLds <= 160 * 1024;
}

int launch_head_bwd(const HeadBwdArgs& a, hipStream_t s) {
  if (a.R <= 0) return 0;
  SND_CHECK_ARG(head_bwd_supported(a.L, a.gh, a.W, a.h1, a.kp1, a.np1, a.kp2, a.np2),
                "head_bwd: unsupported widths (L %d gh %d W %d h1 %d)", a.L, a.gh, a.W, a.h1);
  SND_CHECK_ARG((long long)a.R * a.L * 2 < (1ll << 31), "head_bwd: rows x L beyond the 2 GB buffer range");
  SND_CHECK_ARG(a.rowptr && (a.colidx || a.R == 0) && a.zb && a.edge_part && a.ms && a.eps && a.dz_dec &&
                    a.dJd && a.dms && a.bms_part && a.wmsb_img && a.dh && a.bh_part && a.whb_img && a.ge &&
                    a.g1 && a.b1 && a.p1 && a.x && a.dp1 && a.enc1_part,
                "head_bwd: null operand");
  SND_TRY(head_init_attributes());
  const int nb1 = (a.np1 / 16 + 1) / 2, nb2 = (a.np2 / 16 + 1) / 2;
#define SND_HB(B1)                                   \
  switch (nb2) {                                     \
    case 1: return head_bwd_launch<1, B1, 1>(a, s);  \
    case 2: return head_bwd_launch<1, B1, 2>(a, s);  \
    case 3: return head_bwd_launch<1, B1, 3>(a, s);  \
    default: return head_bwd_launch<1, B1, 4>(a, s); \
  }
  if (nb1 == 1) { SND_HB(1) } else { SND_HB(2) }
#undef SND_HB
}

bool head_fwd_supported(int h1, int f, int gh, int L, int kp1, int np1, int kp2, int np2) {
  if (h1 % 8 || h1 < 8 || h1 > 64 || f < 1 || f > 8) return false;
  if ((kp1 != 32 && kp1 != 64 && kp1 != 128) || (kp2 != 32 && kp2 != 64 && kp2 != 128)) return false;
  if (h1 + 8 > kp1 || gh % 16 || gh < 16 || np1 != gh || np1 > 64 || gh > kp2) return false;
  if ((L != 32 && L != 64) || np2 != 2 * L) return false;
  const FwdLay l64(64, kp1, np1, kp2, np2, L), l128(128, kp1, np1, kp2, np2, L);
  return l128.total <= kHeadDynLds && l64.sx_end <= l64.zt && l128.sx_end <= l128.zt;
}

int launch_head_fwd(const HeadFwdArgs& a, hipStream_t s) {
  if (a.R <= 0) return 0;
  SND_CHECK_ARG(head_fwd_supported(a.h1, a.f, a.gh, a.L, a.kp1, a.np1, a.kp2, a.np2),
                "head_fwd: unsupported widths (h1 %d f %d gh %d L %d)", a.h1, a.f, a.gh, a.L);
  SND_CHECK_ARG(a.npad % 128 == 0 && a.npad >= a.npg && (long long)a.npg * a.ngraphs == a.R,
                "head_fwd: npad %% 128, R = ngraphs x npg");
  SND_CHECK_ARG(a.ldg % 8 == 0 && a.ldg >= a.h1 + 8, "head_fwd: ldg");
  SND_CHECK_ARG((long long)a.R * a.h1 * 2 < (1ll << 31), "head_fwd: rows x h1 beyond the 2 GB buffer range");
  SND_CHECK_ARG(a.rowptr && (a.colidx || a.R == 0) && a.xw1 && a.g1 && a.b1 && a.x && a.ge && a.be && a.p1 &&
                    a.g && a.wh_img && a.bh && a.hh && a.wms_img && a.bms && a.ms && a.z && a.eps_out &&
                    a.zb && a.jrow && a.jt && a.colpart && a.kl_part,
                "head_fwd: null operand");
  SND_TRY(head_init_attributes());
  return head_fwd_dispatch<kHeadRows>(a, s);
}

static int head_init_attributes_once() {
  const void* ks[] = {reinterpret_cast<const void*>(head_fwd_kernel<64, 1, 2>),
                      reinterpret_cast<const void*>(head_fwd_kernel<64, 1, 4>),
                      reinterpret_cast<const void*>(head_fwd_kernel<64, 2, 2>),
                      reinterpret_cast<const void*>(head_fwd_kernel<64, 2, 4>)};
  const void* kb[] = {reinterpret_cast<const void*>(head_bwd_kernel<kHeadBwdRows, 1, 1, 1>),
                      reinterpret_cast<const void*>(head_bwd_kernel<kHeadBwdRows, 1, 1, 2>),
                      reinterpret_cast<const void*>(head_bwd_kernel<kHeadBwdRows, 1, 1, 3>),
                      reinterpret_cast<const void*>(head_bwd_kernel<kHeadBwdRows, 1, 1, 4>),
                      reinterpret_cast<const void*>(head_bwd_kernel<kHeadBwdRows, 1, 2, 1>),
                      reinterpret_cast<const void*>(head_bwd_kernel<kHeadBwdRows, 1, 2, 2>),
                      reinterpret_cast<const void*>(head_bwd_kernel<kHeadBwdRows, 1, 2, 3>),
                      reinterpret_cast<const void*>(head_bwd_kernel<kHeadBwdRows, 1, 2, 4>),
                      reinterpret_cast<const void*>(head_bwd_kernel<64, 1, 1, 1>),
                      reinterpret_cast<const void*>(head_bwd_kernel<64, 1, 1, 2>),
                      reinterpret_cast<const void*>(head_bwd_kernel<64, 1, 1, 3>),
                      reinterpret_cast<const void*>(head_bwd_kernel<64, 1, 1, 4>),
                      reinterpret_cast<const void*>(head_bwd_kernel<64, 1, 2, 1>),
                      reinterpret_cast<const void*>(head_bwd_kernel<64, 1, 2, 2>),
                      reinterpret_cast<const void*>(head_bwd_kernel<64, 1, 2, 3>),
                      reinterpret_cast<const void*>(head_bwd_kernel<64, 1, 2, 4>),
                      reinterpret_cast<const void*>(head_bwd_kernel<kHeadBwdTinyRows, 1, 1, 1>),
                      reinterpret_cast<const void*>(head_bwd_kernel<kHeadBwdTinyRows, 1, 1, 2>),
                      reinterpret_cast<const void*>(head_bwd_kernel<kHeadBwdTinyRows, 1, 1, 3>),
                      reinterpret_cast<const void*>(head_bwd_kernel<kHeadBwdTinyRows, 1, 1, 4>),
                      reinterpret_cast<const void*>(head_bwd_kernel<kHeadBwdTinyRows, 1, 2, 1>),
                      reinterpret_cast<const void*>(head_bwd_kernel<kHeadBwdTinyRows, 1, 2, 2>),
                      reinterpret_cast<const void*>(head_bwd_kernel<kHeadBwdTinyRows, 1, 2, 3>),
                      reinterpret_cast<const void*>(head_bwd_kernel<kHeadBwdTinyRows, 1, 2, 4>)};
  const void* kf[] = {reinterpret_cast<const void*>(enc_front_kernel<1>),
                      reinterpret_cast<const void*>(enc_front_kernel<2>),
                      reinterpret_cast<const void*>(enc_front_kernel<3>),
                      reinterpret_cast<const void*>(enc_front_kernel<4>)};
  for (const void* k : kf) {
    if (hipFuncSetAttribute(k, hipFuncAttributeMaxDynamicSharedMemorySize, 160 * 1024 - 6 * 128 * 4) !=
        hipSuccess) {
      set_error("head: hipFuncSetAttribute failed");
      return SND_ERR_HIP;
    }
  }
  for (const void* k : kb) {
    if (hipFuncSetAttribute(k, hipFuncAttributeMaxDynamicSharedMemorySize, 160 * 1024 - kBwdStaticLds) !=
        hipSuccess) {
      set_error("head: hipFuncSetAttribute failed");
      return SND_ERR_HIP;
    }
  }
  for (const void* k : ks) {
    if (hipFuncSetAttribute(k, hipFuncAttributeMaxDynamicSharedMemorySize, kHeadDynLds) != hipSuccess) {
      set_error("head: hipFuncSetAttribute failed");
      return SND_ERR_HIP;
    }
  }
  return 0;
}

int head_init_attributes() {
  static const int rc = head_init_attributes_once();
  return rc;
}

}
```

snd_vae_amd/csrc/snd_pack.hpp:

```cpp
#pragma once
#include "snd_fast.hpp"

namespace snd {

__host__ __device__ __forceinline__ int img_swz(int row, int kp) {
  return kp >= 128 ? (row & 15) : (kp == 64 ? ((row >> 1) & 7) : 0);
}

__device__ __forceinline__ void pack_chunk_vals(const PackDesc& d, int i, float (&vals)[8]) {
  const int kc = d.kp >> 3;
  const int c = i % kc, tn = i / kc;
  const int n = tn % d.np, t = tn / d.np;
  const int lc = c ^ img_swz(n, d.kp);
#pragma unroll
  for (int j = 0; j < 8; ++j) {
    const int k = 8 * lc + j;
    float val = 0.f;
    for (int si = 0; si < d.nsrc; ++si) {
      const PackSrc& s = d.s[si];
      if (s.mode == 2) {
        if (k == n && k >= s.a0 && k < s.a1) val = 1.f;
        continue;
      }
      int aa, bb, tt;
      if (s.mode == 0) { bb = n - s.n_off + s.b0; aa = k - s.k_off + s.a0; tt = t; }
      else { aa = n - s.n_off + s.a0; bb = k - s.k_off + s.b0; tt = d.T - 1 - t; }
      if (aa >= s.a0 && aa < s.a1 && bb >= s.b0 && bb < s.b1)
        val = s.w[((long long)tt * s.A + aa) * s.B + bb];
    }
    vals[j] = val;
  }
}
__device__ __forceinline__ void pack_chunk_store(const PackDesc& d, int i, const float (&vals)[8]) {
  const int kc = d.kp >> 3;
  const int c = i % kc, tn = i / kc;
  const int n = tn % d.np, t = tn / d.np;
  bf16x8 v;
#pragma unroll
  for (int j = 0; j < 8; ++j) v[j] = (__bf16)vals[j];
  *reinterpret_cast<bf16x8*>(d.dst + ((long long)(t * d.np + n) * d.kp + 8 * c)) = v;
}
__device__ __forceinline__ void pack_chunk(const PackDesc& d, int i) {
  float vals[8];
  pack_chunk_vals(d, i, vals);
  pack_chunk_store(d, i, vals);
}

__host__ __device__ __forceinline__ int pack_chunks(const PackDesc& d) { return d.T * d.np * (d.kp >> 3); }

}
```

Baseline: 38030 graphs/s.

## Hoist and batch global loads to raise memory-level parallelism across kernels

Across several kernels, scalar global loads that were predicated or dependent are turned into unconditional, clamped-index loads issued up front. Parameter staging now reads through pointer arrays, rowptr reads are hoisted before staging, and the CSR gather prefetches the next colidx chunk. Head and front kernels reorder their weight staging so it overlaps with these loads, and they cache BN params in LDS. The intent is to hide global-memory latency. The cost is extra registers and extra LDS, plus new alignment and h1>=4 requirements; a masked partial store path in head_bwd is removed on the basis of that new alignment assumption.

```diff
diff --git a/snd_vae_amd/csrc/snd_fast.hip b/snd_vae_amd/csrc/snd_fast.hip
--- a/snd_vae_amd/csrc/snd_fast.hip
+++ b/snd_vae_amd/csrc/snd_fast.hip
@@ -95,28 +95,50 @@
       glds16(g + ((long long)(t * np + nbase) * kp * 2) + (jj << 10), reinterpret_cast<char*>(ws) + (j << 10));
     }
   }
+  int grp0 = 0, grp1 = 0;
+  if constexpr (EPI == RC_ENC0 && NBH <= 2) {
+    if (a.g_rowptr) {
+      const int grc = min(r0 + (tid >> 3), a.R - 1);
+      grp0 = a.g_rowptr[grc];
+      grp1 = a.g_rowptr[grc + 1];
+    }
+  }
   if (tid < nloc) {
     const int nl = tid, n = nbase + tid;
     const bool cv = n < a.N && a.cols.valid(n) && !(kdbg(a.dbg) & 16);
     const bool pa = n < a.cols.a;
     const int ia = pa ? n : a.cols.logical(n), ib = n - a.cols.offb;
+    const float* zf = reinterpret_cast<const float*>(a.zero);
     auto par = [&](const float* A, const float* Bv) {
-      return !cv || !A ? 0.f : (pa || !Bv ? A[ia] : Bv[ib]);
+      return !cv || !A ? zf : (pa || !Bv ? A + ia : Bv + ib);
     };
-    colp[0][nl] = par(a.bias, a.bias_b);
-    colp[1][nl] = par(a.gamma, a.gamma_b) * kBnC;
-    colp[2][nl] = par(a.beta, a.beta_b);
+    const float* src[7] = {par(a.bias, a.bias_b), par(a.gamma, a.gamma_b), par(a.beta, a.beta_b), zf, zf, zf, zf};
     if constexpr (EPI == RC_ENC1) {
-      colp[3][nl] = (cv && n < a.h) ? a.g2[n] * kBnC : 0.f;
-      colp[4][nl] = (cv && n < a.h) ? a.b2[n] : 0.f;
+      src[3] = (cv && n < a.h) ? a.g2 + n : zf;
+      src[4] = (cv && n < a.h) ? a.b2 + n : zf;
     }
     if constexpr (EPI == RC_ENC0) {
 #pragma unroll
-      for (int k = 0; k < 4; ++k) colp[3 + k][nl] = (cv && k < a.f) ? a.w0[k * a.N + n] : 0.f;
+      for (int k = 0; k < 4; ++k) src[3 + k] = (cv && k < a.f) ? a.w0 + (k * a.N + n) : zf;
     }
     if constexpr (EPI == RC_LIN || EPI == RC_FWD) {
 #pragma unroll
-      for (int k = 0; k < 4; ++k) colp[3 + k][nl] = (cv && k < a.ktail) ? a.wtail[k * a.ldwt + n] : 0.f;
+      for (int k = 0; k < 4; ++k) src[3 + k] = (cv && k < a.ktail) ? a.wtail + (k * a.ldwt + n) : zf;
+    }
+    constexpr int NP = EPI == RC_ENC1 ? 5 : (EPI == RC_ENC0 || EPI == RC_LIN || EPI == RC_FWD ? 7 : 3);
+    float pv[NP];
+#pragma unroll
+    for (int k = 0; k < NP; ++k) pv[k] = *src[k];
+    colp[0][nl] = pv[0];
+    colp[1][nl] = pv[1] * kBnC;
+    colp[2][nl] = pv[2];
+    if constexpr (EPI == RC_ENC1) {
+      colp[3][nl] = pv[3] * kBnC;
+      colp[4][nl] = pv[4];
+    }
+    if constexpr (NP == 7) {
+#pragma unroll
+      for (int k = 0; k < 4; ++k) colp[3 + k][nl] = pv[3 + k];
     }
   }
 
@@ -152,7 +174,7 @@
         float acc8[8] = {0.f, 0.f, 0.f, 0.f, 0.f, 0.f, 0.f, 0.f};
         if (gr < rend) {
           const __amdgpu_buffer_rsrc_t rsx = rows_rsrc(a.x, (long long)a.R * a.ldx * 2);
-          gather_rows16<1>(a.g_colidx, a.g_rowptr[gr], a.g_rowptr[gr + 1], rsx, 2u * a.ldx, sub,
+          gather_rows16<1>(a.g_colidx, grp0, grp1, rsx, 2u * a.ldx, sub,
                            [&](int, const u32x4 (&v)[1], bool) { acc8v(acc8, v[0]); });
         }
         const uint4 o = to_bf16x8(acc8);
@@ -208,9 +230,13 @@
     }
     float ax[4] = {0.f, 0.f, 0.f, 0.f};
     if constexpr (EPI == RC_ENC0) {
-      if (rv)
-#pragma unroll
-        for (int k = 0; k < 4; ++k) if (k < a.f) ax[k] = a.p[(long long)r * a.ldp + k];
+      if (rv && a.f > 0) {
+        float t[4];
+#pragma unroll
+        for (int k = 0; k < 4; ++k) t[k] = a.p[(long long)r * a.ldp + min(k, a.f - 1)];
+#pragma unroll
+        for (int k = 0; k < 4; ++k) ax[k] = k < a.f ? t[k] : 0.f;
+      }
     }
     if constexpr (EPI == RC_LIN || EPI == RC_FWD) {
       if (rv && a.ktail > 0) {
diff --git a/snd_vae_amd/csrc/snd_gather.hpp b/snd_vae_amd/csrc/snd_gather.hpp
--- a/snd_vae_amd/csrc/snd_gather.hpp
+++ b/snd_vae_amd/csrc/snd_gather.hpp
@@ -29,9 +29,14 @@
 template <int NQ, typename Fn>
 __device__ __forceinline__ void gather_rows16(const int* colidx, int s, int e, __amdgpu_buffer_rsrc_t rs,
                                               unsigned row_bytes, int sub, Fn&& fn) {
+  if (s >= e) return;
+  const int last = e - 1;
+  int n0 = colidx[min(s + sub, last)], n1 = colidx[min(s + 8 + sub, last)];
   for (int k0 = s; k0 < e; k0 += 16) {
-    const int id0 = k0 + sub < e ? colidx[k0 + sub] : -1;
-    const int id1 = k0 + 8 + sub < e ? colidx[k0 + 8 + sub] : -1;
+    const int id0 = k0 + sub < e ? n0 : -1;
+    const int id1 = k0 + 8 + sub < e ? n1 : -1;
+    n0 = colidx[min(k0 + 16 + sub, last)];
+    n1 = colidx[min(k0 + 24 + sub, last)];
     int c[16];
     c[0] = bcast8<0>(id0); c[1] = bcast8<1>(id0); c[2] = bcast8<2>(id0); c[3] = bcast8<3>(id0);
     c[4] = bcast8<4>(id0); c[5] = bcast8<5>(id0); c[6] = bcast8<6>(id0); c[7] = bcast8<7>(id0);
diff --git a/snd_vae_amd/csrc/snd_head.hip b/snd_vae_amd/csrc/snd_head.hip
--- a/snd_vae_amd/csrc/snd_head.hip
+++ b/snd_vae_amd/csrc/snd_head.hip
@@ -34,7 +34,7 @@
     sx_end = 2 * HR * (L + 4) * 4;
   }
 };
-constexpr int kHeadStaticLds = 2 * 128 * 4 + 2 * HWMAX * 8;
+constexpr int kHeadStaticLds = 2 * 128 * 4 + 4 * 80 * 4 + 2 * HWMAX * 8;
 constexpr int kHeadDynLds = 160 * 1024 - kHeadStaticLds - 512;
 
 __device__ __forceinline__ void stage_img(const __bf16* src, int bytes, char* dst, int nw) {
@@ -71,11 +71,20 @@
   return reinterpret_cast<bf16x4*>(img + row * kp + (((n0 >> 3) ^ hswz(row, kp)) << 3) + (n0 & 4));
 }
 
+template <int F, int N>
+__device__ __forceinline__ void feat_row(const float* x, int ldx, long long c, float (&v)[N]) {
+  struct __attribute__((packed, aligned(4))) Row { float f[F]; };
+  const Row t = *reinterpret_cast<const Row*>(x + c * ldx);
+#pragma unroll
+  for (int j = 0; j < N; ++j) v[j] = j < F ? t.f[j < F ? j : 0] : 0.f;
+}
+
 template <int HR, int NB1, int NB2>
 __global__ void __launch_bounds__(HR * 8) head_fwd_kernel(HeadFwdArgs a) {
   constexpr int HT = HR * 8, HW = HT / 64, NRB = HR / 16;
   extern __shared__ __attribute__((aligned(16))) char smem[];
   __shared__ float cb1[128], cb2[128];
+  __shared__ float cbn[4][80];
   __shared__ double klw[2 * HWMAX];
   const FwdLay lay(HR, a.kp1, a.np1, a.kp2, a.np2, a.L);
   __bf16* w2s = reinterpret_cast<__bf16*>(smem + lay.w2);
@@ -98,47 +107,67 @@
   const int lr0 = lt * HR;
   const long long gr0 = (long long)gi * a.npg;
 
-  stage_img(a.wh_img, a.np1 * a.kp1 * 2, reinterpret_cast<char*>(w1s), HW);
-  stage_img(a.wms_img, a.np2 * a.kp2 * 2, reinterpret_cast<char*>(w2s), HW);
-  for (int i = tid; i < 128; i += HT) {
-    cb1[i] = i < a.gh ? a.bh[i] : 0.f;
-    cb2[i] = i < 2 * L ? a.bms[i] : 0.f;
-  }
   for (int i = tid; i < HR * a.kp2 / 8; i += HT) reinterpret_cast<uint4*>(hs)[i] = make_uint4(0u, 0u, 0u, 0u);
-
   const int rs = tid >> 3, sub = tid & 7;
   const int lr = lr0 + rs;
   const bool rv = lr < a.npg;
   const long long r = gr0 + lr;
+  const long long rc = gr0 + min(lr, a.npg - 1);
+  const int nch = a.h1 >> 3, kc1 = a.kp1 >> 3;
+  const int xo = (sub == nch) ? 0 : (sub + 8 == nch ? 1 : -1);
+  const int pc = tid & 127;
+  const float bhv = a.bh[min(pc, a.gh - 1)], bmsv = a.bms[min(pc, 2 * L - 1)];
+  const int bc1 = min(tid, a.h1 - 1), bce = min(tid, a.h1 + a.f - 1);
+  const float g1v = a.g1[bc1], b1v = a.b1[bc1], gev = a.ge[bce], bev = a.be[bce];
+  const int rp0 = a.rowptr[rc], rp1 = a.rowptr[rc + 1];
+  float xown[8];
+  switch (a.f) {
+    case 1: feat_row<1, 8>(a.x, a.ldx, rc, xown); break;
+    case 2: feat_row<2, 8>(a.x, a.ldx, rc, xown); break;
+    case 3: feat_row<3, 8>(a.x, a.ldx, rc, xown); break;
+    case 4: feat_row<4, 8>(a.x, a.ldx, rc, xown); break;
+    case 5: feat_row<5, 8>(a.x, a.ldx, rc, xown); break;
+    case 6: feat_row<6, 8>(a.x, a.ldx, rc, xown); break;
+    case 7: feat_row<7, 8>(a.x, a.ldx, rc, xown); break;
+    default: feat_row<8, 8>(a.x, a.ldx, rc, xown); break;
+  }
+  stage_img(a.wh_img, a.np1 * a.kp1 * 2, reinterpret_cast<char*>(w1s), HW);
+  stage_img(a.wms_img, a.np2 * a.kp2 * 2, reinterpret_cast<char*>(w2s), HW);
+  if (tid < 128) {
+    cb1[tid] = tid < a.gh ? bhv : 0.f;
+    cb2[tid] = tid < 2 * L ? bmsv : 0.f;
+  }
+  if (tid < 80) { cbn[0][tid] = g1v; cbn[1][tid] = b1v; cbn[2][tid] = gev; cbn[3][tid] = bev; }
+  __builtin_amdgcn_s_waitcnt(0x0F70);
+  __syncthreads();
+  uint4 gdat = make_uint4(0u, 0u, 0u, 0u), gxv = make_uint4(0u, 0u, 0u, 0u);
+  if (xo >= 0 && rv) {
+    float gv[8];
+#pragma unroll
+    for (int j = 0; j < 8; ++j) {
+      const int c = a.h1 + j;
+      gv[j] = j < a.f ? xown[j] * (cbn[2][c] * kBnC) + cbn[3][c] : 0.f;
+    }
+    gxv = to_bf16x8(gv);
+  }
+
   float acc[8];
 #pragma unroll
   for (int j = 0; j < 8; ++j) acc[j] = 0.f;
   if (rv && !(kdbg(a.dbg) & 1)) {
     const __amdgpu_buffer_rsrc_t rsd = rows_rsrc(a.xw1, (long long)a.R * a.h1 * 2);
-    gather_rows16<1>(a.colidx, a.rowptr[r], a.rowptr[r + 1], rsd, 2u * a.h1, sub,
+    gather_rows16<1>(a.colidx, rp0, rp1, rsd, 2u * a.h1, sub,
                      [&](int, const u32x4 (&v)[1], bool) { acc8v(acc, v[0]); });
   }
-  const int nch = a.h1 >> 3, kc1 = a.kp1 >> 3;
-  uint4 gdat = make_uint4(0u, 0u, 0u, 0u), gxv = make_uint4(0u, 0u, 0u, 0u);
   if (sub < nch) {
     float gv[8];
 #pragma unroll
     for (int j = 0; j < 8; ++j) {
       const int c = 8 * sub + j;
-      const float b1 = lrelu(acc[j]) * (a.g1[c] * kBnC) + a.b1[c];
-      gv[j] = b1 * (a.ge[c] * kBnC) + a.be[c];
+      const float b1 = lrelu(acc[j]) * (cbn[0][c] * kBnC) + cbn[1][c];
+      gv[j] = b1 * (cbn[2][c] * kBnC) + cbn[3][c];
     }
     gdat = to_bf16x8(gv);
-  }
-  const int xo = (sub == nch) ? 0 : (sub + 8 == nch ? 1 : -1);
-  if (xo >= 0 && rv) {
-    float gv[8];
-#pragma unroll
-    for (int j = 0; j < 8; ++j) {
-      const int c = a.h1 + j;
-      gv[j] = j < a.f ? a.x[r * a.ldx + j] * (a.ge[c] * kBnC) + a.be[c] : 0.f;
-    }
-    gxv = to_bf16x8(gv);
   }
   {
     const bool d0 = sub < nch, x0 = xo == 0, x1 = xo == 1;
@@ -148,7 +177,6 @@
     if (sub < kc1) *reinterpret_cast<uint4*>(gs + rs * a.kp1 + ((sub ^ hswz(rs, a.kp1)) << 3)) = v0;
     if (sub + 8 < kc1) *reinterpret_cast<uint4*>(gs + rs * a.kp1 + (((sub + 8) ^ hswz(rs, a.kp1)) << 3)) = v1;
   }
-  __builtin_amdgcn_s_waitcnt(0x0F70);
   __syncthreads();
   if (rv && !(kdbg(a.dbg) & 8)) {
     if (sub < nch) {
@@ -342,15 +370,9 @@
   }
   const int r0 = t * HR;
 
-  stage_img(a.wmsb_img, a.np1 * a.kp1 * 2, reinterpret_cast<char*>(w1s), HW);
-  stage_img(a.whb_img, a.np2 * a.kp2 * 2, reinterpret_cast<char*>(w2s), HW);
   for (int i = tid; i < HR * a.kp2 / 8; i += HT) reinterpret_cast<uint4*>(dh_img)[i] = make_uint4(0u, 0u, 0u, 0u);
-  for (int n = tid; n < 128; n += HT) {
-    const bool cv = n < a.W;
-    colp[1][n] = cv ? a.ge[n] * kBnC : 0.f;
-    colp[3][n] = (cv && n < a.h1) ? a.g1[n] * kBnC : 0.f;
-    colp[4][n] = (cv && n < a.h1) ? a.b1[n] : 0.f;
-  }
+  const int pn = min(tid, 127);
+  const float pge = a.ge[min(pn, a.W - 1)], pg1 = a.g1[min(pn, a.h1 - 1)], pb1 = a.b1[min(pn, a.h1 - 1)];
 
   {
     const int rs = tid >> 3, sub = tid & 7;
@@ -370,14 +392,24 @@
 #pragma unroll
       for (int j = 0; j < 8; ++j) ej[q][j] = 0.f;
     }
+    const int rc = min(r, a.R - 1);
+    const int rp0 = a.rowptr[rc], rp1 = a.rowptr[rc + 1];
     if (rv)
 #pragma unroll
       for (int q = 0; q < NQ; ++q)
         if (qv[q]) zi[q] = *reinterpret_cast<const u32x4*>(a.zb + (long long)r * L + 64 * q + 8 * sub);
+    stage_img(a.wmsb_img, a.np1 * a.kp1 * 2, reinterpret_cast<char*>(w1s), HW);
+    stage_img(a.whb_img, a.np2 * a.kp2 * 2, reinterpret_cast<char*>(w2s), HW);
+    if (tid < 128) {
+      const bool cv = tid < a.W;
+      colp[1][tid] = cv ? pge * kBnC : 0.f;
+      colp[3][tid] = (cv && tid < a.h1) ? pg1 * kBnC : 0.f;
+      colp[4][tid] = (cv && tid < a.h1) ? pb1 : 0.f;
+    }
     const float pw = a.pos_weight;
     if (rv && !(kdbg(a.dbg) & 1)) {
       const __amdgpu_buffer_rsrc_t rsd = rows_rsrc(a.zb, (long long)a.R * L * 2);
-      gather_rows16<NQ>(a.colidx, a.rowptr[r], a.rowptr[r + 1], rsd, 2u * L, sub,
+      gather_rows16<NQ>(a.colidx, rp0, rp1, rsd, 2u * L, sub,
                         [&](int, const u32x4 (&v)[NQ], bool valid) {
         float zj[NQ][8], dot = 0.f;
 #pragma unroll
@@ -413,17 +445,25 @@
       if (rv && qv[q]) {
         const float* msr = a.ms + (long long)r * L2;
         const long long ie = (long long)r * L + c0;
+        float4 muq[2], lsq[2], epq[2], djq[2], ddq[2];
 #pragma unroll
         for (int h = 0; h < 2; ++h) {
-          const float4 mu = *reinterpret_cast<const float4*>(msr + c0 + 4 * h);
-          const float4 ls = *reinterpret_cast<const float4*>(msr + L + c0 + 4 * h);
-          const float4 ep = *reinterpret_cast<const float4*>(a.eps + ie + 4 * h);
-          float4 dj = *reinterpret_cast<const float4*>(a.dJd + ie + 4 * h);
-          for (int sx = 0; sx < a.nextra; ++sx) {
+          muq[h] = *reinterpret_cast<const float4*>(msr + c0 + 4 * h);
+          lsq[h] = *reinterpret_cast<const float4*>(msr + L + c0 + 4 * h);
+          epq[h] = *reinterpret_cast<const float4*>(a.eps + ie + 4 * h);
+          djq[h] = *reinterpret_cast<const float4*>(a.dJd + ie + 4 * h);
+          ddq[h] = *reinterpret_cast<const float4*>(a.dz_dec + ie + 4 * h);
+        }
+        for (int sx = 0; sx < a.nextra; ++sx) {
+#pragma unroll
+          for (int h = 0; h < 2; ++h) {
             const float4 e = *reinterpret_cast<const float4*>(a.dJd_extra + (long long)sx * a.R * L + ie + 4 * h);
-            dj.x += e.x; dj.y += e.y; dj.z += e.z; dj.w += e.w;
+            djq[h].x += e.x; djq[h].y += e.y; djq[h].z += e.z; djq[h].w += e.w;
           }
-          const float4 dd = *reinterpret_cast<const float4*>(a.dz_dec + ie + 4 * h);
+        }
+#pragma unroll
+        for (int h = 0; h < 2; ++h) {
+          const float4 mu = muq[h], ls = lsq[h], ep = epq[h], dj = djq[h], dd = ddq[h];
           const float m4[4] = {mu.x, mu.y, mu.z, mu.w}, l4[4] = {ls.x, ls.y, ls.z, ls.w};
           const float e4[4] = {ep.x, ep.y, ep.z, ep.w}, j4[4] = {dj.x, dj.y, dj.z, dj.w};
           const float d4[4] = {dd.x, dd.y, dd.z, dd.w};
@@ -498,17 +538,30 @@
   }
   f32x4 ypf[NB2];
   unsigned cvm[NB2];
-#pragma unroll
-  for (int i = 0; i < NB2; ++i) {
-    ypf[i] = f32x4{0.f, 0.f, 0.f, 0.f};
-    cvm[i] = 0u;
-    const int nb = NB2 * half + i;
-#pragma unroll
-    for (int e = 0; e < 4; ++e) {
-      const int n = 16 * nb + 4 * lg + e;
-      if (nb < (a.np2 >> 4) && n < a.W) {
-        cvm[i] |= 1u << e;
-        if (vrow) ypf[i][e] = n < a.h1 ? a.p1[(long long)r * a.h1 + n] : a.x[(long long)r * a.ldx + (n - a.h1)];
+  {
+    const long long rcl = min(r, a.R - 1);
+    const int fx = a.W - a.h1;
+    f32x4 pq[NB2];
+    float xq[NB2][4];
+#pragma unroll
+    for (int i = 0; i < NB2; ++i) {
+      const int n0 = 16 * (NB2 * half + i) + 4 * lg;
+      pq[i] = *reinterpret_cast<const f32x4*>(a.p1 + rcl * a.h1 + min(n0, a.h1 - 4));
+#pragma unroll
+      for (int e = 0; e < 4; ++e) xq[i][e] = a.x[rcl * a.ldx + min(max(n0 + e - a.h1, 0), max(fx - 1, 0))];
+    }
+#pragma unroll
+    for (int i = 0; i < NB2; ++i) {
+      ypf[i] = f32x4{0.f, 0.f, 0.f, 0.f};
+      cvm[i] = 0u;
+      const int nb = NB2 * half + i;
+#pragma unroll
+      for (int e = 0; e < 4; ++e) {
+        const int n = 16 * nb + 4 * lg + e;
+        if (nb < (a.np2 >> 4) && n < a.W) {
+          cvm[i] |= 1u << e;
+          if (vrow) ypf[i][e] = n < a.h1 ? pq[i][e] : xq[i][e];
+        }
       }
     }
   }
@@ -561,9 +614,6 @@
 #pragma unroll
           for (int e = 0; e < 4; ++e) v4[e] = (__bf16)o[e];
           *reinterpret_cast<bf16x4*>(op) = v4;
-        } else {
-#pragma unroll
-          for (int e = 0; e < 4; ++e) if (sm >> e & 1u) op[e] = (__bf16)o[e];
         }
       }
 #pragma unroll
@@ -601,6 +651,51 @@
   return 0;
 }
 
+template <int F>
+__device__ __forceinline__ void front_ax(const float* x, int ldx, const int* colidx, int s, int e, int sub,
+                                         int rc, float (&ax)[4], float (&xown)[4]) {
+  feat_row<F, 4>(x, ldx, rc, xown);
+  if (s >= e) return;
+  const int last = e - 1;
+  int c[4];
+#pragma unroll
+  for (int u = 0; u < 4; ++u) c[u] = colidx[min(s + sub + 8 * u, last)];
+#pragma unroll
+  for (int u = 0; u < 4; ++u) asm volatile("" : "+v"(c[u]));
+  float v[4][4];
+#pragma unroll
+  for (int u = 0; u < 4; ++u) feat_row<F, 4>(x, ldx, c[u], v[u]);
+#pragma unroll
+  for (int u = 0; u < 4; ++u)
+#pragma unroll
+    for (int j = 0; j < F; ++j) asm volatile("" : "+v"(v[u][j]));
+#pragma unroll
+  for (int t = 0; t < 2; ++t) {
+    const int k = s + sub + 16 * t;
+    const bool p0 = k < e, p1 = k + 8 < e;
+#pragma unroll
+    for (int j = 0; j < 4; ++j) {
+      const float v0 = p0 ? v[2 * t][j] : 0.f, v1 = p1 ? v[2 * t + 1][j] : 0.f;
+      ax[j] += p1 ? v0 + v1 : v0;
+    }
+  }
+  int k = s + sub + 32;
+  for (; k + 8 < e; k += 16) {
+    const int c0 = colidx[k], c1 = colidx[k + 8];
+    float v0[4], v1[4];
+    feat_row<F, 4>(x, ldx, c0, v0);
+    feat_row<F, 4>(x, ldx, c1, v1);
+#pragma unroll
+    for (int j = 0; j < 4; ++j) ax[j] += v0[j] + v1[j];
+  }
+  if (k < e) {
+    float v0[4];
+    feat_row<F, 4>(x, ldx, colidx[k], v0);
+#pragma unroll
+    for (int j = 0; j < 4; ++j) ax[j] += v0[j];
+  }
+}
+
 template <int NB>
 __global__ void __launch_bounds__(1024) enc_front_kernel(FrontArgs a) {
   const int tid = threadIdx.x;
@@ -621,49 +716,48 @@
   __bf16* himg = reinterpret_cast<__bf16*>(smem + a.np1 * a.kp1 * 2);
   const int r0 = blockIdx.x * 128;
   const int K1 = a.h0 + a.f;
-  for (int i = tid; i < a.h0; i += 1024) {
-#pragma unroll
-    for (int q = 0; q < 4; ++q) sp[q][i] = q < a.f ? a.w0[q * a.h0 + i] : 0.f;
-    sp[4][i] = a.g0[i] * kBnC;
-    sp[5][i] = a.b0[i];
-  }
-  __syncthreads();
-  const int kc = a.kp1 >> 3;
-  const bool w1one = a.np1 * kc <= 1024;
-  float w1v[8];
-  if (w1one && tid < a.np1 * kc) {
-    const int c = tid % kc, n = tid / kc;
-    const int lc = c ^ img_swz(n, a.kp1);
-#pragma unroll
-    for (int j = 0; j < 8; ++j) {
-      const int k = 8 * lc + j;
-      w1v[j] = (k < K1 && n < a.n1) ? a.w1[k * a.n1 + n] : 0.f;
-    }
-  }
   const int rs = tid >> 3, sub = tid & 7;
   const int r = r0 + rs;
   const bool rv = r < a.R;
-  float ax[4] = {0.f, 0.f, 0.f, 0.f};
-  if (rv) {
-    const int s = a.rowptr[r], e = a.rowptr[r + 1];
-    int k = s + sub;
-    for (; k + 8 < e; k += 16) {
-      const int c0 = a.colidx[k], c1 = a.colidx[k + 8];
-      float v0[4], v1[4];
-#pragma unroll
-      for (int j = 0; j < 4; ++j) {
-        v0[j] = j < a.f ? a.x[(long long)c0 * a.ldx + j] : 0.f;
-        v1[j] = j < a.f ? a.x[(long long)c1 * a.ldx + j] : 0.f;
-      }
-#pragma unroll
-      for (int j = 0; j < 4; ++j) ax[j] += v0[j] + v1[j];
-    }
-    if (k < e) {
-      const int c0 = a.colidx[k];
-#pragma unroll
-      for (int j = 0; j < 4; ++j) ax[j] += j < a.f ? a.x[(long long)c0 * a.ldx + j] : 0.f;
-    }
-  }
+  const int fm = a.f - 1;
+  const int pi = min(tid, a.h0 - 1);
+  float spv[6];
+#pragma unroll
+  for (int q = 0; q < 4; ++q) spv[q] = a.w0[min(q, fm) * a.h0 + pi];
+  spv[4] = a.g0[pi];
+  spv[5] = a.b0[pi];
+  const int kc = a.kp1 >> 3;
+  const bool w1one = a.np1 * kc <= 1024;
+  const int wc = tid % kc, wn = tid / kc;
+  const int wlc = wc ^ img_swz(wn, a.kp1);
+  float w1v[8];
+  if (w1one) {
+    const int nn = min(wn, a.n1 - 1);
+#pragma unroll
+    for (int j = 0; j < 8; ++j) w1v[j] = a.w1[min(8 * wlc + j, K1 - 1) * a.n1 + nn];
+  }
+  const int rc = min(r, a.R - 1);
+  const int s = a.rowptr[rc], e1 = a.rowptr[rc + 1];
+  const int e = rv ? e1 : s;
+  float ax[4] = {0.f, 0.f, 0.f, 0.f}, xown[4];
+  switch (a.f) {
+    case 1: front_ax<1>(a.x, a.ldx, a.colidx, s, e, sub, rc, ax, xown); break;
+    case 2: front_ax<2>(a.x, a.ldx, a.colidx, s, e, sub, rc, ax, xown); break;
+    case 3: front_ax<3>(a.x, a.ldx, a.colidx, s, e, sub, rc, ax, xown); break;
+    default: front_ax<4>(a.x, a.ldx, a.colidx, s, e, sub, rc, ax, xown); break;
+  }
+#pragma unroll
+  for (int j = 0; j < 4; ++j) asm volatile("" : "+v"(ax[j]));
+  if (w1one)
+#pragma unroll
+    for (int j = 0; j < 8; ++j) asm volatile("" : "+v"(w1v[j]));
+  if (tid < a.h0) {
+#pragma unroll
+    for (int q = 0; q < 4; ++q) sp[q][tid] = q < a.f ? spv[q] : 0.f;
+    sp[4][tid] = spv[4] * kBnC;
+    sp[5][tid] = spv[5];
+  }
+  __syncthreads();
 #pragma unroll
   for (int j = 0; j < 4; ++j) ax[j] = row8_sum(ax[j]);
   const int nch = a.h0 >> 3, kc1 = a.kp1 >> 3;
@@ -684,7 +778,7 @@
   if (xo >= 0 && rv) {
     float xv[8];
 #pragma unroll
-    for (int j = 0; j < 8; ++j) xv[j] = j < a.f ? a.x[(long long)r * a.ldx + j] : 0.f;
+    for (int j = 0; j < 8; ++j) xv[j] = (j < 4 && j < a.f) ? xown[j & 3] : 0.f;
     hx = to_bf16x8(xv);
   }
   {
@@ -697,22 +791,21 @@
   }
   if (w1one) {
     if (tid < a.np1 * kc) {
-      const int c = tid % kc, n = tid / kc;
       bf16x8 v;
 #pragma unroll
-      for (int j = 0; j < 8; ++j) v[j] = (__bf16)w1v[j];
-      *reinterpret_cast<bf16x8*>(wimg + n * a.kp1 + 8 * c) = v;
+      for (int j = 0; j < 8; ++j) v[j] = (__bf16)((8 * wlc + j < K1 && wn < a.n1) ? w1v[j] : 0.f);
+      *reinterpret_cast<bf16x8*>(wimg + wn * a.kp1 + 8 * wc) = v;
     }
   } else {
     for (int i = tid; i < a.np1 * kc; i += 1024) {
       const int c = i % kc, n = i / kc;
       const int lc = c ^ img_swz(n, a.kp1);
+      float wv[8];
+#pragma unroll
+      for (int j = 0; j < 8; ++j) wv[j] = a.w1[min(8 * lc + j, K1 - 1) * a.n1 + min(n, a.n1 - 1)];
       bf16x8 v;
 #pragma unroll
-      for (int j = 0; j < 8; ++j) {
-        const int k = 8 * lc + j;
-        v[j] = (__bf16)((k < K1 && n < a.n1) ? a.w1[k * a.n1 + n] : 0.f);
-      }
+      for (int j = 0; j < 8; ++j) v[j] = (__bf16)((8 * lc + j < K1 && n < a.n1) ? wv[j] : 0.f);
       *reinterpret_cast<bf16x8*>(wimg + n * a.kp1 + 8 * c) = v;
     }
   }
@@ -793,7 +886,7 @@
 bool head_bwd_supported(int L, int gh, int W, int h1, int kp1, int np1, int kp2, int np2) {
   if ((L != 16 && L != 32 && L != 64) || kp1 != 2 * L) return false;
   if (gh % 16 || gh < 16 || np1 != gh || np1 > 64 || gh > kp2 || (kp2 != 32 && kp2 != 64 && kp2 != 128)) return false;
-  if (W > 128 || np2 != (int)round_up(W, 16) || h1 % 4 || h1 > W) return false;
+  if (W > 128 || np2 != (int)round_up(W, 16) || h1 % 4 || h1 < 4 || h1 > W) return false;
   return BwdLay(kp1, np1, kp2, np2, L).total + kBwdStaticLds <= 160 * 1024;
 }
 
@@ -802,6 +895,7 @@
   SND_CHECK_ARG(head_bwd_supported(a.L, a.gh, a.W, a.h1, a.kp1, a.np1, a.kp2, a.np2),
                 "head_bwd: unsupported widths (L %d gh %d W %d h1 %d)", a.L, a.gh, a.W, a.h1);
   SND_CHECK_ARG((long long)a.R * a.L * 2 < (1ll << 31), "head_bwd: rows x L beyond the 2 GB buffer range");
+  SND_CHECK_ARG((reinterpret_cast<uintptr_t>(a.p1) & 15) == 0, "head_bwd: P1 must be 16-byte aligned");
   SND_CHECK_ARG(a.rowptr && (a.colidx || a.R == 0) && a.zb && a.edge_part && a.ms && a.eps && a.dz_dec &&
                     a.dJd && a.dms && a.bms_part && a.wmsb_img && a.dh && a.bh_part && a.whb_img && a.ge &&
                     a.g1 && a.b1 && a.p1 && a.x && a.dp1 && a.enc1_part,
diff --git a/snd_vae_amd/csrc/snd_pack.hpp b/snd_vae_amd/csrc/snd_pack.hpp
--- a/snd_vae_amd/csrc/snd_pack.hpp
+++ b/snd_vae_amd/csrc/snd_pack.hpp
@@ -13,22 +13,31 @@
   const int n = tn % d.np, t = tn / d.np;
   const int lc = c ^ img_swz(n, d.kp);
 #pragma unroll
-  for (int j = 0; j < 8; ++j) {
-    const int k = 8 * lc + j;
-    float val = 0.f;
-    for (int si = 0; si < d.nsrc; ++si) {
-      const PackSrc& s = d.s[si];
-      if (s.mode == 2) {
-        if (k == n && k >= s.a0 && k < s.a1) val = 1.f;
-        continue;
+  for (int j = 0; j < 8; ++j) vals[j] = 0.f;
+  for (int si = 0; si < d.nsrc; ++si) {
+    const PackSrc& s = d.s[si];
+    if (s.mode == 2) {
+#pragma unroll
+      for (int j = 0; j < 8; ++j) {
+        const int k = 8 * lc + j;
+        if (k == n && k >= s.a0 && k < s.a1) vals[j] = 1.f;
       }
+      continue;
+    }
+    if (s.A <= 0 || s.B <= 0) continue;
+    bool in[8];
+    float wv[8];
+#pragma unroll
+    for (int j = 0; j < 8; ++j) {
+      const int k = 8 * lc + j;
       int aa, bb, tt;
       if (s.mode == 0) { bb = n - s.n_off + s.b0; aa = k - s.k_off + s.a0; tt = t; }
       else { aa = n - s.n_off + s.a0; bb = k - s.k_off + s.b0; tt = d.T - 1 - t; }
-      if (aa >= s.a0 && aa < s.a1 && bb >= s.b0 && bb < s.b1)
-        val = s.w[((long long)tt * s.A + aa) * s.B + bb];
+      in[j] = aa >= s.a0 && aa < s.a1 && bb >= s.b0 && bb < s.b1;
+      wv[j] = s.w[in[j] ? ((long long)tt * s.A + aa) * s.B + bb : 0ll];
     }
-    vals[j] = val;
+#pragma unroll
+    for (int j = 0; j < 8; ++j) vals[j] = in[j] ? wv[j] : vals[j];
   }
 }
 __device__ __forceinline__ void pack_chunk_store(const PackDesc& d, int i, const float (&vals)[8]) {
```

Measured after the change: 38800 graphs/s (median of 6 runs). 1.02x the previous value.
